# felipeagc/sycl-ray-tracer

Hardware: AMD Instinct MI355X
Metric: Mrays/s (higher is better)
Workload: dtype f32

## Files before the change

sycl-ray-tracer_amd/csrc/rt_bounce.h:

```cpp
#pragma once
#include "rt_device.h"

namespace rt {

RT_DEV f3 ray_dir(const RayState& r) { return mk3(h2f(r.dir[0]), h2f(r.dir[1]), h2f(r.dir[2])); }

template <bool FROM_TRAV = false, class Sink = NoSink>
RT_DEV bool shade_bounce(const SceneDev& S, uint32_t& rng, RayState& r, const Hit& h, f3& result, const Trav* T = nullptr, const ShadeTables* tab = nullptr,
                         long long* ck = nullptr, const Sink& sink = Sink{}) {
    f3 org = FROM_TRAV ? T->o : r.org;
    f3 dir = FROM_TRAV ? T->d : ray_dir(r);
    f3 att = mk3(h2f(r.att[0]), h2f(r.att[1]), h2f(r.att[2]));
    f3 rad = mk3(h2f(r.rad[0]), h2f(r.rad[1]), h2f(r.rad[2]));
    const bool done = FROM_TRAV ? shade_hit<true>(S, *tab, rng, h, org, dir, att, rad, result, ck, sink) : shade_hit<false>(S, ShadeTables{}, rng, h, org, dir, att, rad, result, nullptr, sink);
    r.org = org;
    r.dir[0] = f2h(dir.x), r.dir[1] = f2h(dir.y), r.dir[2] = f2h(dir.z);
    r.att[0] = f2h(att.x), r.att[1] = f2h(att.y), r.att[2] = f2h(att.z);
    r.rad[0] = f2h(rad.x), r.rad[1] = f2h(rad.y), r.rad[2] = f2h(rad.z);
    return done;
}

RT_DEV void origin_skip_none(const TravStack& stack) { *lds_at(skip_word_addr(stack)) = (int32_t)kSkipNone; }
RT_DEV SkipRec skip_entry(const SkipRec* at) {
    const u32x4* ep = reinterpret_cast<const u32x4*>(at);
    const u32x4 a = ep[0], b = ep[1];
    SkipRec e;
    e.ref = a.x, e.n[0] = __uint_as_float(a.y), e.n[1] = __uint_as_float(a.z), e.n[2] = __uint_as_float(a.w);
    e.p[0] = __uint_as_float(b.x), e.p[1] = __uint_as_float(b.y), e.p[2] = __uint_as_float(b.z), e.a = b.w;
    return e;
}
RT_DEV void origin_skip(const SceneDev& S, uint32_t tri, const Trav& T, const TravStack& stack) {
    const SkipRec e = skip_entry(S.skip + (tri == kNoTri ? 0u : tri));
    const float o[3] = {T.o.x, T.o.y, T.o.z}, d[3] = {T.d.x, T.d.y, T.d.z};
    const uint32_t w = origin_skip_word(e, o, d);
    *lds_at(skip_word_addr(stack)) = (int32_t)(tri == kNoTri ? kSkipNone : w);
}

RT_DEV bool roulette(uint32_t& rng, RayState& r) {
    const float qx = h2f(r.att[0]), qy = h2f(r.att[1]), qz = h2f(r.att[2]);
    const float p = __builtin_fminf(__builtin_fmaxf(__builtin_fmaxf(qx, __builtin_fmaxf(qy, qz)), 0.05f), 1.0f);
    const float u = rng_next(rng);
    if (!(u < p)) return false;
    r.att[0] = f2h(qx / p), r.att[1] = f2h(qy / p), r.att[2] = f2h(qz / p);
    return true;
}

}
```

sycl-ray-tracer_amd/csrc/rt_device.h:

```cpp
#pragma once
#include <hip/hip_runtime.h>

#include "../../include/rt_mi355x.h"
#include "rt_types.h"

namespace rt {

#define RT_DEV __device__ __forceinline__

struct f3 {
    float x, y, z;
};
RT_DEV f3 mk3(float x, float y, float z) { return f3{x, y, z}; }
RT_DEV f3 operator+(f3 a, f3 b) { return mk3(a.x + b.x, a.y + b.y, a.z + b.z); }
RT_DEV f3 operator-(f3 a, f3 b) { return mk3(a.x - b.x, a.y - b.y, a.z - b.z); }
RT_DEV f3 operator-(f3 a) { return mk3(-a.x, -a.y, -a.z); }
RT_DEV f3 operator*(f3 a, f3 b) { return mk3(a.x * b.x, a.y * b.y, a.z * b.z); }
RT_DEV f3 operator*(float s, f3 a) { return mk3(s * a.x, s * a.y, s * a.z); }
RT_DEV f3 operator*(f3 a, float s) { return mk3(a.x * s, a.y * s, a.z * s); }
RT_DEV float dot3(f3 a, f3 b) { return (a.x * b.x + a.y * b.y) + a.z * b.z; }
RT_DEV f3 cross3(f3 a, f3 b) {
    return mk3(a.y * b.z - a.z * b.y, a.z * b.x - a.x * b.z, a.x * b.y - a.y * b.x);
}
RT_DEV float rcp_rn(float x) {
    const uint32_t t = __float_as_uint(x) + __float_as_uint(x);
    const bool ok = t - 0x01000000u < 0xFC000000u;
    if (__builtin_expect(__builtin_amdgcn_ballot_w64(!ok) == 0ull, 1)) {
        const float y = __builtin_amdgcn_rcpf(x);
        return __builtin_fmaf(__builtin_fmaf(-x, y, 1.0f), y, y);
    }
    return 1.0f / x;
}
RT_DEV float inv_sqrt2(float x) {
    const bool ok = __float_as_uint(x) - 0x0C800000u < 0x73000000u;
    if (__builtin_expect(__builtin_amdgcn_ballot_w64(!ok) == 0ull, 1)) {
        const float r = __builtin_amdgcn_rsqf(x);
        float g = x * r, h = 0.5f * r;
        const float e = __builtin_fmaf(-h, g, 0.5f);
        g = __builtin_fmaf(g, e, g), h = __builtin_fmaf(h, e, h);
        const float s = __builtin_fmaf(__builtin_fmaf(-g, g, x), h, g);
        const float y = __builtin_amdgcn_rcpf(s);
        return __builtin_fmaf(__builtin_fmaf(-s, y, 1.0f), y, y);
    }
    return 1.0f / __builtin_sqrtf(x);
}
RT_DEV f3 normalize3(f3 a) {
    const float inv = inv_sqrt2(dot3(a, a));
    return mk3(a.x * inv, a.y * inv, a.z * inv);
}
RT_DEV float clamp01(float x) { return __builtin_fminf(__builtin_fmaxf(x, 0.0f), 1.0f); }

RT_DEV uint16_t f2h(float f) {
    asm("" : "+v"(f));
    _Float16 h = (_Float16)f;
    return __builtin_bit_cast(uint16_t, h);
}
RT_DEV float h2f(uint16_t b) { return (float)__builtin_bit_cast(_Float16, b); }

RT_DEV float rng_next(uint32_t& a) {
    uint32_t x = a;
    x ^= x << 13;
    x ^= x >> 17;
    x ^= x << 5;
    a = x;
    return (float)x * (1.0f / 4294967296.0f);
}
RT_DEV float rng_range(uint32_t& a, float mn, float mx) { return mn + (mx - mn) * rng_next(a); }
RT_DEV f3 rng_unit_vector(uint32_t& a) {
    float x = rng_range(a, -1.0f, 1.0f);
    float y = rng_range(a, -1.0f, 1.0f);
    float z = rng_range(a, -1.0f, 1.0f);
    return normalize3(mk3(x, y, z));
}

RT_DEV uint32_t pixel_seed(int x, int y, int w, int h, uint32_t seed_mode) {
    if (seed_mode == RT_SEED_MEGAKERNEL) {
        uint32_t h8 = (uint32_t)((h + 7) / 8) * 8u;
        return (uint32_t)x * h8 + (uint32_t)y;
    }
    return (uint32_t)x + (uint32_t)y * (uint32_t)w;
}

RT_DEV int tile_global_row(const TileDev& t, int local_row) {
    uint32_t strip = (uint32_t)local_row / t.strip_rows;
    uint32_t within = (uint32_t)local_row % t.strip_rows;
    return (int)((strip * t.world + t.rank) * t.strip_rows + within);
}

struct RayState {
    f3 org;
    uint16_t dir[3], att[3], rad[3];
};

RT_DEV RayState camera_ray(const CameraDev& c, int x, int y, uint32_t& rng) {
    f3 p00 = mk3(c.pixel00[0], c.pixel00[1], c.pixel00[2]);
    f3 du = mk3(c.du[0], c.du[1], c.du[2]);
    f3 dv = mk3(c.dv[0], c.dv[1], c.dv[2]);
    f3 center = mk3(c.center[0], c.center[1], c.center[2]);
    f3 pixel_center = (p00 + ((float)x * du)) + ((float)y * dv);
    float px = -0.5f + rng_next(rng);
    float py = -0.5f + rng_next(rng);
    f3 jitter = (px * du) + (py * dv);
    f3 pixel_sample = pixel_center + jitter;
    f3 d = pixel_sample - center;
    RayState r;
    r.org = center;
    r.dir[0] = f2h(d.x), r.dir[1] = f2h(d.y), r.dir[2] = f2h(d.z);
    r.att[0] = r.att[1] = r.att[2] = 0x3C00;
    r.rad[0] = r.rad[1] = r.rad[2] = 0;
    return r;
}

struct Hit {
    float t, u, v;
    uint32_t tri;
};

RT_DEV float dot3f(f3 a, f3 b) { return __builtin_fmaf(a.z, b.z, __builtin_fmaf(a.y, b.y, a.x * b.x)); }
RT_DEV f3 cross3f(f3 a, f3 b) {
    return mk3(__builtin_fmaf(a.y, b.z, -(a.z * b.y)), __builtin_fmaf(a.z, b.x, -(a.x * b.z)), __builtin_fmaf(a.x, b.y, -(a.y * b.x)));
}
RT_DEV void tri_test_regs(float4 a, float4 b, float2 c, f3 o, f3 d, Hit& best) {
    const f3 v0 = mk3(a.x, a.y, a.z), e1 = mk3(a.w, b.x, b.y), e2 = mk3(b.z, b.w, c.x);
    const uint32_t gidx = __float_as_uint(c.y);
    const f3 p = cross3f(d, e2);
    const float det = dot3f(e1, p);
    if (!(det != 0.0f)) return;
    const f3 tv = o - v0;
    const f3 q = cross3f(tv, e1);
    const float sgn = det < 0.0f ? -1.0f : 1.0f;
    const float un0 = dot3f(tv, p), vn0 = dot3f(d, q);
    const float un = un0 * sgn, vn = vn0 * sgn;
    if (!(un >= 0.0f && vn >= 0.0f && un + vn <= __builtin_fabsf(det))) return;
    const float inv = rcp_rn(det);
    const float t = dot3f(e2, q) * inv;
    if (!(t > kTNear)) return;
    if (t < best.t || (t == best.t && gidx < best.tri)) {
        best.t = t;
        best.u = un0 * inv;
        best.v = vn0 * inv;
        best.tri = gidx;
    }
}
typedef float f4a8 __attribute__((ext_vector_type(4), aligned(8)));
typedef float f2a8 __attribute__((ext_vector_type(2), aligned(8)));
RT_DEV float4 tri_ld4(const uint8_t* p) {
    const f4a8 v = *reinterpret_cast<const f4a8*>(p);
    return make_float4(v.x, v.y, v.z, v.w);
}
RT_DEV float2 tri_ld2(const uint8_t* p) {
    const f2a8 v = *reinterpret_cast<const f2a8*>(p);
    return make_float2(v.x, v.y);
}
RT_DEV void tri_test(const uint8_t* __restrict__ tr, f3 o, f3 d, Hit& best) {
    tri_test_regs(tri_ld4(tr), tri_ld4(tr + 16), tri_ld2(tr + 32), o, d, best);
}

constexpr int32_t kTravDone = (int32_t)0x80000000;
#if defined(RT_DEVELOPER_KNOBS) && defined(RT_VOTE_INNER) && defined(RT_VOTE_LEAF)
constexpr uint32_t kVoteInner = RT_VOTE_INNER, kVoteLeaf = RT_VOTE_LEAF;
#else
constexpr uint32_t kVoteInner = 3u, kVoteLeaf = 4u;
#endif
struct Trav {
    f3 o, d;
    float ix, iy, iz;
    float ox, oy, oz;
    Hit best;
    int32_t cur;
    uint32_t sp;
};

struct TravStack;
RT_DEV uint32_t stack_base(const TravStack& st);
RT_DEV void trav_begin(Trav& T, f3 o, f3 d, const TravStack& st) {
    T.o = o, T.d = d;
    T.best.t = __builtin_huge_valf();
    T.best.u = T.best.v = 0.0f;
    T.best.tri = kNoTri;
    const float kTiny = 1e-30f;
    const float dx = __builtin_fabsf(d.x) < kTiny ? __builtin_copysignf(kTiny, d.x) : d.x;
    const float dy = __builtin_fabsf(d.y) < kTiny ? __builtin_copysignf(kTiny, d.y) : d.y;
    const float dz = __builtin_fabsf(d.z) < kTiny ? __builtin_copysignf(kTiny, d.z) : d.z;
    T.ix = __builtin_amdgcn_rcpf(dx), T.iy = __builtin_amdgcn_rcpf(dy), T.iz = __builtin_amdgcn_rcpf(dz);
    T.ox = -o.x * T.ix, T.oy = -o.y * T.iy, T.oz = -o.z * T.iz;
    T.cur = 0;
    T.sp = stack_base(st);
}

constexpr int kLdsStack = 12;
typedef __attribute__((address_space(3))) int32_t lds_i32;
struct TravStack {
    uint32_t base;
    int32_t* spill;
    uint32_t pitch;
};
RT_DEV uint32_t stack_base(const TravStack& st) { return st.base + st.pitch; }
RT_DEV lds_i32* lds_at(uint32_t addr) { return (lds_i32*)(size_t)addr; }
RT_DEV uint32_t skip_word_addr(const TravStack& st) { return st.base + (uint32_t)kLdsStack * st.pitch; }
RT_DEV bool stack_shallow(const TravStack& st, const Trav& T, uint32_t pushes) { return T.sp <= st.base + ((uint32_t)kLdsStack - pushes) * st.pitch; }
RT_DEV void trav_pop_lds(Trav& T, const TravStack& st) {
    T.sp -= st.pitch;
    T.cur = *lds_at(T.sp);
}
RT_DEV void stk_push(const TravStack& st, Trav& T, int32_t v) {
    const uint32_t e = (T.sp - st.base) / st.pitch;
    if (e < (uint32_t)kLdsStack) *lds_at(T.sp) = v;
    else st.spill[e - (uint32_t)kLdsStack] = v;
    T.sp += st.pitch;
}
RT_DEV void trav_pop(Trav& T, const TravStack& st) {
    T.sp -= st.pitch;
    const uint32_t e = (T.sp - st.base) / st.pitch;
    T.cur = e < (uint32_t)kLdsStack ? *lds_at(T.sp) : st.spill[e - (uint32_t)kLdsStack];
}

typedef uint32_t u32x4 __attribute__((ext_vector_type(4)));
typedef uint32_t u32x2 __attribute__((ext_vector_type(2)));
typedef __attribute__((address_space(3))) u32x4 lds_u32x4;
struct TopTree {
    lds_u32x4* w0;
    lds_u32x4* w1;
    lds_u32x4* w2;
    lds_u32x4* ch;
    int32_t count;
};
RT_DEV void top_tree_fill(const SceneDev& S, u32x4* w0, u32x4* w1, u32x4* w2, u32x4* ch, int32_t count) {
    for (int32_t i = (int32_t)threadIdx.x; i < count; i += (int32_t)blockDim.x) {
        const u32x4* np = reinterpret_cast<const u32x4*>(S.nodes + i);
        w0[i] = np[0];
        w1[i] = np[1];
        w2[i] = np[2];
        ch[i] = np[3];
    }
}

typedef unsigned long long lmask;
RT_DEV lmask lanes(bool c) { return __builtin_amdgcn_ballot_w64(c); }
RT_DEV uint32_t lane_rank(lmask m) { return __builtin_amdgcn_mbcnt_hi((uint32_t)(m >> 32), __builtin_amdgcn_mbcnt_lo((uint32_t)m, 0u)); }
RT_DEV float sel(lmask m, float a, float b) {
    float d;
    asm("v_cndmask_b32_e64 %0, %1, %2, %3" : "=v"(d) : "v"(a), "v"(b), "s"(m));
    return d;
}
RT_DEV uint32_t sel(lmask m, uint32_t a, uint32_t b) {
    uint32_t d;
    asm("v_cndmask_b32_e64 %0, %1, %2, %3" : "=v"(d) : "v"(a), "v"(b), "s"(m));
    return d;
}
RT_DEV int32_t sel(lmask m, int32_t a, int32_t b) { return (int32_t)sel(m, (uint32_t)a, (uint32_t)b); }
RT_DEV bool in_mask(lmask m) { return __builtin_amdgcn_inverse_ballot_w64(m); }
RT_DEV uint32_t count(lmask m) { return (uint32_t)__builtin_popcountll(m); }

struct TravSigns {
    lmask nx, ny, nz;
};

RT_DEV float ub0(uint32_t w) { return (float)(w & 0xffu); }
RT_DEV float ub1(uint32_t w) { return (float)((w >> 8) & 0xffu); }
RT_DEV float ub2(uint32_t w) { return (float)((w >> 16) & 0xffu); }
RT_DEV float ub3(uint32_t w) { return (float)(w >> 24); }

struct WaveStats {
    uint32_t inner_steps = 0, inner_lanes = 0, leaf_steps = 0, leaf_lanes = 0;
    uint32_t shade_rounds = 0, shade_lanes = 0, live_lane_steps = 0, top_lanes = 0;
};
RT_DEV TravSigns trav_signs(const Trav& T) { return TravSigns{lanes(T.ix < 0.0f), lanes(T.iy < 0.0f), lanes(T.iz < 0.0f)}; }
template <bool SKIP = false, bool MISS_KEYS = false>
RT_DEV void trav_inner(const SceneDev& S, Trav& T, const TravStack& stack, const TopTree& top, const TravSigns& sg) {
    const float inf = __builtin_huge_valf();
    uint32_t skip = kSkipNone;
    if (SKIP) skip = (uint32_t)*lds_at(skip_word_addr(stack));
    float k0, k1, k2, k3;
    u32x4 w0, w1, w2, chw;
    if (T.cur < top.count * 64) {
        const uint32_t o = (uint32_t)T.cur >> 2;
        w0 = *(lds_u32x4*)(size_t)((uint32_t)(size_t)top.w0 + o), w1 = *(lds_u32x4*)(size_t)((uint32_t)(size_t)top.w1 + o);
        w2 = *(lds_u32x4*)(size_t)((uint32_t)(size_t)top.w2 + o), chw = *(lds_u32x4*)(size_t)((uint32_t)(size_t)top.ch + o);
    } else {
        asm volatile("global_load_dwordx4 %0, %4, %5\n\t"
                     "global_load_dwordx4 %1, %4, %5 offset:16\n\t"
                     "global_load_dwordx4 %2, %4, %5 offset:32\n\t"
                     "global_load_dwordx4 %3, %4, %5 offset:48"
                     : "=&v"(w0), "=&v"(w1), "=&v"(w2), "=&v"(chw)
                     : "v"((uint32_t)T.cur), "s"(S.nodes)
                     : "memory");
    }
    asm volatile("s_waitcnt vmcnt(1)" : "+v"(w0), "+v"(w1), "+v"(w2));
    const float ax = __uint_as_float(w0.w) * T.ix;
    const float ay = __uint_as_float(w2.z) * T.iy;
    const float az = __uint_as_float(w2.w) * T.iz;
    const float bx = __builtin_fmaf(__uint_as_float(w0.x), T.ix, T.ox);
    const float by = __builtin_fmaf(__uint_as_float(w0.y), T.iy, T.oy);
    const float bz = __builtin_fmaf(__uint_as_float(w0.z), T.iz, T.oz);
    const lmask nx = sg.nx, ny = sg.ny, nz = sg.nz;
    const uint32_t qnx = sel(nx, w1.x, w1.y), qfx = sel(nx, w1.y, w1.x);
    const uint32_t qny = sel(ny, w1.z, w1.w), qfy = sel(ny, w1.w, w1.z);
    const uint32_t qnz = sel(nz, w2.x, w2.y), qfz = sel(nz, w2.y, w2.x);
    lmask h0 = 0ull, h1 = 0ull, h2 = 0ull, h3 = 0ull;
#define RT_CHILD(K, H, CVT, CW)                                                                           \
    {                                                                                                    \
        const float tn = __builtin_fmaxf(__builtin_fmaxf(__builtin_fmaf(CVT(qnx), ax, bx), __builtin_fmaf(CVT(qny), ay, by)), \
                                         __builtin_fmaxf(__builtin_fmaf(CVT(qnz), az, bz), 0.0f));       \
         \
         \
         \
        const float fx = __builtin_fmaf(CVT(qfx), ax, bx), fy = __builtin_fmaf(CVT(qfy), ay, by), fz = __builtin_fmaf(CVT(qfz), az, bz); \
        const float tf = SKIP ? __builtin_fminf(__builtin_fminf(__builtin_fminf(fx, fy), fz), T.best.t)  \
                              : __builtin_fminf(__builtin_fminf(fx, fy), __builtin_fminf(fz, T.best.t)); \
        if (SKIP) H = lanes(tn <= tf) & lanes(CW != skip), K = MISS_KEYS ? sel(H, inf, tn) : tn;         \
        else K = sel(lanes(tn <= tf), inf, tn);                                                          \
    }
    if (SKIP) asm volatile("s_waitcnt vmcnt(0)" : "+v"(chw));
    RT_CHILD(k0, h0, ub0, chw.x)
    RT_CHILD(k1, h1, ub1, chw.y)
    RT_CHILD(k2, h2, ub2, chw.z)
    RT_CHILD(k3, h3, ub3, chw.w)
#undef RT_CHILD
#define RT_CE(KA, CA, KB, CB)                                                        \
    {                                                                               \
        const lmask sw = lanes(KB < KA);                                            \
        const float ka = sel(sw, KA, KB), kb = sel(sw, KB, KA);                     \
        const int32_t ca = sel(sw, CA, CB), cb = sel(sw, CB, CA);                   \
        KA = ka, KB = kb, CA = ca, CB = cb;                                         \
    }
    if (!SKIP) asm volatile("s_waitcnt vmcnt(0)" : "+v"(chw));
    int32_t c0 = (int32_t)chw.x, c1 = (int32_t)chw.y, c2 = (int32_t)chw.z, c3 = (int32_t)chw.w;
    if (SKIP) {
#define RT_CE_M(KA, HA, CA, KB, HB, CB)                                              \
    {                                                                               \
        const lmask sw = MISS_KEYS ? lanes(KB < KA) : HB & (~HA | lanes(KB < KA));  \
        KA = sel(sw, KA, KB);                                                       \
        const int32_t ca = sel(sw, CA, CB), cb = sel(sw, CB, CA);                   \
        CA = ca, CB = cb;                                                           \
        const lmask lo = HA | HB, hi = HA & HB;                                     \
        HA = lo, HB = hi;                                                           \
    }
        RT_CE_M(k0, h0, c0, k1, h1, c1)
        RT_CE_M(k2, h2, c2, k3, h3, c3)
        RT_CE_M(k0, h0, c0, k2, h2, c2)
#undef RT_CE_M
        if (lanes(!stack_shallow(stack, T, 3u)) == 0ull) {
            *lds_at(T.sp) = c3;
            T.sp = sel(h3, T.sp, T.sp + stack.pitch);
            *lds_at(T.sp) = c2;
            T.sp = sel(h2, T.sp, T.sp + stack.pitch);
            *lds_at(T.sp) = c1;
            T.sp = sel(h1, T.sp, T.sp + stack.pitch);
            if (in_mask(h0)) T.cur = c0;
            else trav_pop_lds(T, stack);
        } else {
            if (in_mask(h3)) stk_push(stack, T, c3);
            if (in_mask(h2)) stk_push(stack, T, c2);
            if (in_mask(h1)) stk_push(stack, T, c1);
            if (in_mask(h0)) T.cur = c0;
            else trav_pop(T, stack);
        }
        return;
    }
    RT_CE(k0, c0, k1, c1)
    RT_CE(k2, c2, k3, c3)
    RT_CE(k0, c0, k2, c2)
#undef RT_CE
    const bool descend = k0 < inf;
    if (lanes(!stack_shallow(stack, T, 3u)) == 0ull) {
        *lds_at(T.sp) = c3;
        T.sp = sel(lanes(k3 < inf), T.sp, T.sp + stack.pitch);
        *lds_at(T.sp) = c2;
        T.sp = sel(lanes(k2 < inf), T.sp, T.sp + stack.pitch);
        *lds_at(T.sp) = c1;
        T.sp = sel(lanes(k1 < inf), T.sp, T.sp + stack.pitch);
        if (descend) T.cur = c0;
        else trav_pop_lds(T, stack);
    } else {
        if (k3 < inf) stk_push(stack, T, c3);
        if (k2 < inf) stk_push(stack, T, c2);
        if (k1 < inf) stk_push(stack, T, c1);
        if (descend) T.cur = c0;
        else trav_pop(T, stack);
    }
}

template <bool BATCH>
RT_DEV void trav_leaf(const SceneDev& S, Trav& T, const TravStack& stack) {
    const uint32_t code = (uint32_t)~T.cur;
    const uint32_t first = code >> 2, rem = code & 3u;
    if (BATCH) {
        static_assert(kMaxLeafTris == 2 && kTriBytes == 40, "the whole-leaf step reads a leaf as 80 contiguous bytes");
        const uint8_t* p4 = S.tris + (size_t)first * kTriBytes;
        const float4 l0 = tri_ld4(p4), l1 = tri_ld4(p4 + 16), l2 = tri_ld4(p4 + 32), l3 = tri_ld4(p4 + 48), l4 = tri_ld4(p4 + 64);
        const bool two = rem != 0u;
        tri_test_regs(l0, l1, make_float2(l2.x, l2.y), T.o, T.d, T.best);
        if (__ballot(two) != 0ull) {
            if (two) tri_test_regs(make_float4(l2.z, l2.w, l3.x, l3.y), make_float4(l3.z, l3.w, l4.x, l4.y), make_float2(l4.z, l4.w), T.o, T.d, T.best);
        }
        if (lanes(!stack_shallow(stack, T, 0u)) == 0ull) trav_pop_lds(T, stack);
        else trav_pop(T, stack);
    } else {
        tri_test(S.tris + (size_t)first * kTriBytes, T.o, T.d, T.best);
        if (rem) T.cur = ~(int32_t)(((first + 1u) << 2) | (rem - 1u));
        else trav_pop(T, stack);
    }
}

struct TravClasses {
    lmask inner, leaf;
};
RT_DEV lmask trav_done(const Trav& T) { return lanes(T.cur == kTravDone); }
RT_DEV TravClasses trav_classes(const Trav& T) { return TravClasses{lanes(T.cur >= 0), lanes((uint32_t)T.cur > (uint32_t)kTravDone)}; }
RT_DEV TravClasses trav_classes(const Trav& T, lmask done) {
    const lmask inner = lanes(T.cur >= 0);
    return TravClasses{inner, lanes(true) & ~(inner | done)};
}
template <bool STATS = false, bool LEAF_BATCH = false, bool SKIP = false, bool MISS_KEYS = false>
RT_DEV uint32_t trav_step_wave(const SceneDev& S, Trav& T, const TravStack& stack, const TopTree& top, const TravSigns& sg, const TravClasses& c, WaveStats* ws = nullptr) {
    const uint32_t ni = count(c.inner), nl = count(c.leaf);
    if (ni * kVoteInner >= nl * kVoteLeaf && !(LEAF_BATCH && nl >= 64u)) {
        if (STATS && ni) ws->inner_steps++, ws->inner_lanes += ni, ws->top_lanes += count(c.inner & lanes(T.cur < (SKIP ? top.count : kTopNodes) * 64));
        if (in_mask(c.inner)) trav_inner<SKIP, MISS_KEYS>(S, T, stack, top, sg);
    } else {
        if (STATS) ws->leaf_steps++, ws->leaf_lanes += nl;
        if (in_mask(c.leaf)) trav_leaf<LEAF_BATCH>(S, T, stack);
    }
    return ni + nl;
}
template <bool STATS = false, bool LEAF_BATCH = false, bool SKIP = false, bool MISS_KEYS = false>
RT_DEV uint32_t trav_step_wave(const SceneDev& S, Trav& T, const TravStack& stack, const TopTree& top, const TravSigns& sg, WaveStats* ws = nullptr) {
    return trav_step_wave<STATS, LEAF_BATCH, SKIP, MISS_KEYS>(S, T, stack, top, sg, trav_classes(T), ws);
}

RT_DEV Hit intersect(const SceneDev& S, f3 o, f3 d, const TravStack& stack, const TopTree& top) {
    Trav T;
    trav_begin(T, o, d, stack);
    const TravSigns sg = trav_signs(T);
    while (trav_step_wave(S, T, stack, top, sg)) {}
    return T.best;
}

RT_DEV bool near_zero3(f3 e) {
    const float s = 1e-8f;
    return (__builtin_fabsf(e.x) < s) && (__builtin_fabsf(e.y) < s) && (__builtin_fabsf(e.z) < s);
}
RT_DEV float length_squared3(f3 v) {
    float l = __builtin_sqrtf(dot3(v, v));
    return l * l;
}
RT_DEV f3 reflect3(f3 v, f3 n) { return v - (2.0f * dot3(v, n)) * n; }
RT_DEV f3 refract3(f3 uv, f3 n, float etai_over_etat) {
    float cos_theta = __builtin_fminf(dot3(-uv, n), 1.0f);
    f3 r_out_perp = etai_over_etat * (uv + cos_theta * n);
    f3 r_out_parallel = (-__builtin_sqrtf(__builtin_fabsf(1.0f - length_squared3(r_out_perp)))) * n;
    return r_out_perp + r_out_parallel;
}
RT_DEV float schlick(float cosine, float ref_idx) {
    float r0 = (1.0f - ref_idx) / (1.0f + ref_idx);
    r0 = r0 * r0;
    float x = 1.0f - cosine;
    float x2 = x * x;
    float x5 = (x2 * x2) * x;
    return r0 + (1.0f - r0) * x5;
}
RT_DEV float unorm8_to_float(uint32_t b) {
    const float x = (float)b, r = 1.0f / 255.0f;
    const float q = x * r;
    return __builtin_fmaf(__builtin_fmaf(-q, 255.0f, x), r, q);
}

RT_DEV bool albedo_is_texture(const MatRec& m) { return (m.type == RT_MAT_DIFFUSE || m.type == RT_MAT_METALLIC) && m.tex_kind != RT_TEX_COLOR; }
RT_DEV uint32_t albedo_fetch(const SceneDev& S, const MatRec& m, float u, float v) {
    float fu = u - __builtin_floorf(u);
    float fv = v - __builtin_floorf(v);
    int iu = (int)__builtin_floorf(fu * 512.0f);
    int iv = (int)__builtin_floorf(fv * 512.0f);
    iu = iu < 0 ? 0 : (iu > 511 ? 511 : iu);
    iv = iv < 0 ? 0 : (iv > 511 ? 511 : iv);
    return *reinterpret_cast<const uint32_t*>(S.tex + (((size_t)m.tex_layer * 512u + (size_t)iv) * 512u + (size_t)iu) * 4u);
}
RT_DEV f3 albedo_decode(uint32_t texel) {
    return mk3(unorm8_to_float(texel & 0xffu), unorm8_to_float((texel >> 8) & 0xffu), unorm8_to_float((texel >> 16) & 0xffu));
}
RT_DEV f3 albedo(const SceneDev& S, const MatRec& m, float u, float v) {
    if (m.tex_kind == RT_TEX_COLOR) return mk3(m.color[0], m.color[1], m.color[2]);
    float fu = u - __builtin_floorf(u);
    float fv = v - __builtin_floorf(v);
    int iu = (int)__builtin_floorf(fu * 512.0f);
    int iv = (int)__builtin_floorf(fv * 512.0f);
    iu = iu < 0 ? 0 : (iu > 511 ? 511 : iu);
    iv = iv < 0 ? 0 : (iv > 511 ? 511 : iv);
    const uint32_t texel = *reinterpret_cast<const uint32_t*>(
        S.tex + (((size_t)m.tex_layer * 512u + (size_t)iv) * 512u + (size_t)iu) * 4u);
    return mk3(unorm8_to_float(texel & 0xffu), unorm8_to_float((texel >> 8) & 0xffu), unorm8_to_float((texel >> 16) & 0xffu));
}

template <bool PRE = false>
RT_DEV bool scatter(const SceneDev& S, const MatRec& m, uint32_t& rng, f3 dir, f3 normal, float u, float v,
                    f3& out_dir, f3& out_att, uint32_t texel = 0) {
    if (m.type == RT_MAT_DIFFUSE || m.type == RT_MAT_METALLIC) {
        const bool diffuse = m.type == RT_MAT_DIFFUSE;
        const f3 unit = rng_unit_vector(rng);
        const f3 reflected = reflect3(dir, normal);
        const f3 base = diffuse ? normal : reflected;
        const f3 offs = diffuse ? unit : m.roughness * unit;
        out_dir = base + offs;
        if (diffuse && near_zero3(dir)) out_dir = normal;
        if (PRE) out_att = m.tex_kind == RT_TEX_COLOR ? mk3(m.color[0], m.color[1], m.color[2]) : albedo_decode(texel);
        else out_att = albedo(S, m, u, v);
        return diffuse ? true : dot3(out_dir, normal) > 0.0f;
    }
    if (m.type == RT_MAT_DIELECTRIC) {
        out_att = mk3(1.0f, 1.0f, 1.0f);
        bool front_face = dot3(dir, normal) < 0.0f;
        f3 n = front_face ? normal : -normal;
        float ratio = front_face ? (1.0f / m.ior) : m.ior;
        f3 unit_direction = normalize3(dir);
        float cos_theta = __builtin_fminf(dot3(-unit_direction, n), 1.0f);
        float sin_theta = __builtin_sqrtf(1.0f - cos_theta * cos_theta);
        bool reflect_it = ratio * sin_theta > 1.0f;
        if (!reflect_it) reflect_it = schlick(cos_theta, ratio) > rng_range(rng, 0.0f, 1.0f);
        out_dir = reflect_it ? reflect3(unit_direction, n) : refract3(unit_direction, n, ratio);
        return true;
    }
    out_dir = mk3(0.0f, 0.0f, 0.0f);
    out_att = mk3(0.0f, 0.0f, 0.0f);
    return false;
}

struct ShadeTables {
    lds_u32x4* nm;
    lds_u32x4* mat;
    uint32_t n_nm, n_mat;
};
RT_DEV void shade_tables_fill(const SceneDev& S, u32x4* nm, u32x4* mat) {
    const u32x4* in = reinterpret_cast<const u32x4*>(S.inst);
    for (uint32_t i = threadIdx.x; i < S.lds_nm * 3u; i += blockDim.x) nm[i] = in[i];
    for (uint32_t i = threadIdx.x; i < S.lds_mats; i += blockDim.x) {
        const u32x4* mp = reinterpret_cast<const u32x4*>(S.mats + i);
        const u32x4 m0 = mp[0], m1 = mp[1], m2 = mp[2];
        u32x4 a, b;
        a.x = m0.x | (m0.y << 8) | (m1.y << 16), a.y = m0.z, a.z = m0.w, a.w = m1.x;
        b.x = m1.z, b.y = m1.w, b.z = m2.x, b.w = m0.x == RT_MAT_DIELECTRIC ? m2.z : m2.y;
        mat[2u * i] = a, mat[2u * i + 1u] = b;
    }
}

#ifdef RT_ROUND_STAMPS
#define RT_STAMP_AFTER(ck, i, VAL)                                                     \
    do {                                                                              \
        if (ck) {                                                                     \
            asm volatile("" ::"v"(VAL));                                              \
            const long long n_ = (long long)__builtin_readcyclecounter();             \
            (ck)[i] += n_ - (ck)[7];                                                  \
            (ck)[7] = n_;                                                             \
        }                                                                             \
    } while (0)
#else
#define RT_STAMP_AFTER(ck, i, VAL) do { } while (0)
#endif
struct NoSink {};
template <class Sink> struct is_no_sink { static constexpr bool value = false; };
template <> struct is_no_sink<NoSink> { static constexpr bool value = true; };
template <bool USE_TAB = false, class Sink = NoSink>
RT_DEV bool shade_hit(const SceneDev& S, const ShadeTables& tab, uint32_t& rng, const Hit& h, f3& org, f3& dir, f3& att, f3& rad, f3& result,
                      long long* ck = nullptr, const Sink& sink = Sink{}) {
    if (h.tri == kNoTri) {
        if constexpr (is_no_sink<Sink>::value) result = att * (mk3(S.sky[0], S.sky[1], S.sky[2]) + rad);
        else sink(att * (mk3(S.sky[0], S.sky[1], S.sky[2]) + rad));
        return true;
    }
    const float4* sp = reinterpret_cast<const float4*>(S.shade + h.tri);
    const float4 s0 = sp[0], s1 = sp[1], s2 = sp[2], s3 = sp[3];
    const f3 d = normalize3(dir);
    const f3 n0 = mk3(s0.x, s0.y, s0.z), n1 = mk3(s0.w, s1.x, s1.y), n2 = mk3(s1.z, s1.w, s2.x);
    const float uv0x = s2.y, uv0y = s2.z, uv1x = s2.w, uv1y = s3.x, uv2x = s3.y, uv2y = s3.z;
    const uint32_t iw = __float_as_uint(s3.w);
    RT_STAMP_AFTER(ck, 1, iw);
    bool lds = false;
    if (USE_TAB) lds = __builtin_amdgcn_ballot_w64(!((iw & kPackedInstMask) < tab.n_nm && (iw >> kPackedInstBits) < tab.n_mat)) == 0ull;
    MatRec mat;
    if (USE_TAB && __builtin_expect(lds, 1)) {
        const uint32_t at = (iw >> kPackedInstBits) * 2u;
        const u32x4 a = tab.mat[at], b = tab.mat[at + 1u];
        mat.type = a.x & 0xffu, mat.tex_kind = (a.x >> 8) & 0xffu, mat.tex_layer = a.x >> 16;
        mat.color[0] = __uint_as_float(a.y), mat.color[1] = __uint_as_float(a.z), mat.color[2] = __uint_as_float(a.w);
        mat.emissive[0] = __uint_as_float(b.x), mat.emissive[1] = __uint_as_float(b.y), mat.emissive[2] = __uint_as_float(b.z);
        mat.roughness = mat.ior = __uint_as_float(b.w);
    } else {
        const InstRec* inst = S.inst + (S.packed_mat ? (iw & kPackedInstMask) : iw);
        const u32x4* mp = reinterpret_cast<const u32x4*>(S.mats + (S.packed_mat ? (iw >> kPackedInstBits) : inst->material));
        const u32x4 m0 = mp[0], m1 = mp[1], m2 = mp[2];
        mat.type = m0.x, mat.tex_kind = m0.y, mat.color[0] = __uint_as_float(m0.z), mat.color[1] = __uint_as_float(m0.w);
        mat.color[2] = __uint_as_float(m1.x), mat.tex_layer = m1.y, mat.emissive[0] = __uint_as_float(m1.z), mat.emissive[1] = __uint_as_float(m1.w);
        mat.emissive[2] = __uint_as_float(m2.x), mat.roughness = __uint_as_float(m2.y), mat.ior = __uint_as_float(m2.z);
    }
    const float bx = h.u, by = h.v;
    const float w = (1.0f - bx) - by;
    const float tu = (w * uv0x + bx * uv1x) + by * uv2x;
    const float tv = (w * uv0y + bx * uv1y) + by * uv2y;
    uint32_t texel;
    {
        float fu = tu - __builtin_floorf(tu);
        float fv = tv - __builtin_floorf(tv);
        int iu = (int)__builtin_floorf(fu * 512.0f);
        int iv = (int)__builtin_floorf(fv * 512.0f);
        iu = iu < 0 ? 0 : (iu > 511 ? 511 : iu);
        iv = iv < 0 ? 0 : (iv > 511 ? 511 : iv);
        const uint8_t* ta = S.tex + (((size_t)mat.tex_layer * 512u + (size_t)iv) * 512u + (size_t)iu) * 4u;
        if (!albedo_is_texture(mat)) ta = reinterpret_cast<const uint8_t*>(sp);
        texel = *reinterpret_cast<const uint32_t*>(ta);
        RT_STAMP_AFTER(ck, 2, ta);
    }
    const bool emits = mat.type == RT_MAT_DIFFUSE || mat.type == RT_MAT_METALLIC;
    rad = rad + (emits ? mk3(mat.emissive[0], mat.emissive[1], mat.emissive[2]) : mk3(0.0f, 0.0f, 0.0f));
    const f3 vn = normalize3((w * n0 + bx * n1) + by * n2);
    float nm[9];
    if (USE_TAB && __builtin_expect(lds, 1)) {
        const uint32_t at = (iw & kPackedInstMask) * 3u;
        const u32x4 a = tab.nm[at], b = tab.nm[at + 1u];
        const uint32_t c = *reinterpret_cast<__attribute__((address_space(3))) const uint32_t*>(tab.nm + at + 2u);
        nm[0] = __uint_as_float(a.x), nm[1] = __uint_as_float(a.y), nm[2] = __uint_as_float(a.z), nm[3] = __uint_as_float(a.w);
        nm[4] = __uint_as_float(b.x), nm[5] = __uint_as_float(b.y), nm[6] = __uint_as_float(b.z), nm[7] = __uint_as_float(b.w);
        nm[8] = __uint_as_float(c);
    } else {
        const InstRec* inst = S.inst + (S.packed_mat ? (iw & kPackedInstMask) : iw);
        u32x4 a, b;
        uint32_t c;
        asm volatile("global_load_dwordx4 %0, %3, off\n\t"
                     "global_load_dwordx4 %1, %3, off offset:16\n\t"
                     "global_load_dword %2, %3, off offset:32\n\t"
                     "s_waitcnt vmcnt(0)"
                     : "=&v"(a), "=&v"(b), "=&v"(c)
                     : "v"(inst)
                     : "memory");
        nm[0] = __uint_as_float(a.x), nm[1] = __uint_as_float(a.y), nm[2] = __uint_as_float(a.z), nm[3] = __uint_as_float(a.w);
        nm[4] = __uint_as_float(b.x), nm[5] = __uint_as_float(b.y), nm[6] = __uint_as_float(b.z), nm[7] = __uint_as_float(b.w);
        nm[8] = __uint_as_float(c);
    }
    const f3 g = mk3((nm[0] * vn.x + nm[3] * vn.y) + nm[6] * vn.z, (nm[1] * vn.x + nm[4] * vn.y) + nm[7] * vn.z,
                     (nm[2] * vn.x + nm[5] * vn.y) + nm[8] * vn.z);
    const f3 normal = normalize3(g);
    RT_STAMP_AFTER(ck, 3, normal.x);
    f3 sdir, satt;
#ifdef RT_SCATTER_PRIO
    __builtin_amdgcn_s_setprio(RT_SCATTER_PRIO);
#endif
    const bool scattered = scatter<true>(S, mat, rng, d, normal, tu, tv, sdir, satt, texel);
    RT_STAMP_AFTER(ck, 4, satt.x);
    if (scattered) {
        org = mk3(org.x + dir.x * h.t, org.y + dir.y * h.t, org.z + dir.z * h.t);
        dir = sdir;
        att = att * satt;
        return false;
    }
    if constexpr (is_no_sink<Sink>::value) result = att * rad;
    else sink(att * rad);
    return true;
}

RT_DEV uint8_t to_unorm8(float c) { return (uint8_t)__builtin_rintf(clamp01(c) * 255.0f); }

#define RT_TRAVERSAL_LDS(BLOCK) RT_TRAVERSAL_LDS_(BLOCK, kTopNodes, 0)
#define RT_TRAVERSAL_LDS_SKIP(BLOCK, ON)                                                               \
    RT_TRAVERSAL_LDS_(BLOCK, (ON) ? kTopNodes - (int)(BLOCK) / 16 : kTopNodes, (ON) ? 1 : 0)           \
    if (ON) lds_stack[kLdsStack * (BLOCK) + threadIdx.x] = (int32_t)kSkipNone;
#define RT_TRAVERSAL_LDS_(BLOCK, NTOP, EXTRA)                                                          \
    __shared__ u32x4 top_all[4 * (NTOP)];  \
    u32x4 *const top_w0 = top_all, *const top_w1 = top_all + (NTOP), *const top_w2 = top_all + 2 * (NTOP), *const top_ch = top_all + 3 * (NTOP); \
    __shared__ int32_t lds_stack[(kLdsStack + (EXTRA)) * (BLOCK)];                                     \
    int32_t spill[kStackSize - kLdsStack];                                                             \
    const int32_t top_count = (int32_t)S.n_nodes < (NTOP) ? (int32_t)S.n_nodes : (NTOP);               \
    top_tree_fill(S, top_w0, top_w1, top_w2, top_ch, top_count);                                       \
    __syncthreads();                                                                                   \
    const TopTree top{(lds_u32x4*)top_w0, (lds_u32x4*)top_w1, (lds_u32x4*)top_w2, (lds_u32x4*)top_ch, top_count}; \
    const TravStack stack{(uint32_t)(size_t)(lds_i32*)(lds_stack + threadIdx.x), spill, 4u * (BLOCK)}; \
    lds_stack[threadIdx.x] = kTravDone;

#define RT_SHADE_LDS                                                                                   \
    __shared__ u32x4 shade_nm[3 * kLdsNm], shade_mat[2 * kLdsMats];                                    \
    shade_tables_fill(S, shade_nm, shade_mat);                                                         \
    const ShadeTables tab{(lds_u32x4*)shade_nm, (lds_u32x4*)shade_mat, S.lds_nm, S.lds_mats};


}
```

sycl-ray-tracer_amd/csrc/rt_kernels.h:

```cpp
#pragma once
#include <cstddef>

#include "rt_bounce.h"
#include "rt_device.h"
#include "rt_launch.h"

namespace rt {

RT_DEV void queue_store(const QueueDev& q, uint32_t slot, uint32_t id, const RayState& r) {
    q.org_id[slot] = make_float4(r.org.x, r.org.y, r.org.z, __uint_as_float(id));
    q.a[slot] = make_uint2((uint32_t)r.dir[0] | ((uint32_t)r.dir[1] << 16), (uint32_t)r.dir[2] | ((uint32_t)r.att[0] << 16));
    q.b[slot] = make_uint2((uint32_t)r.att[1] | ((uint32_t)r.att[2] << 16), (uint32_t)r.rad[0] | ((uint32_t)r.rad[1] << 16));
    q.c[slot] = r.rad[2];
}
RT_DEV uint32_t queue_load(const QueueDev& q, uint32_t slot, RayState& r) {
    const float4 o = q.org_id[slot];
    const uint2 a = q.a[slot], b = q.b[slot];
    const uint16_t c = q.c[slot];
    r.org = mk3(o.x, o.y, o.z);
    r.dir[0] = (uint16_t)a.x, r.dir[1] = (uint16_t)(a.x >> 16), r.dir[2] = (uint16_t)a.y;
    r.att[0] = (uint16_t)(a.y >> 16), r.att[1] = (uint16_t)b.x, r.att[2] = (uint16_t)(b.x >> 16);
    r.rad[0] = (uint16_t)b.y, r.rad[1] = (uint16_t)(b.y >> 16), r.rad[2] = c;
    return __float_as_uint(o.w);
}

RT_DEV uint32_t wave_sum_u32(uint32_t v) {
#pragma unroll
    for (int off = 32; off > 0; off >>= 1) v += __shfl_down(v, off, 64);
    return v;
}
RT_DEV unsigned long long wave_sum_u64(uint32_t v) {
    return (unsigned long long)wave_sum_u32(v & 0xFFFFu) + ((unsigned long long)wave_sum_u32(v >> 16) << 16);
}

RT_DEV void wave_stats_flush(const WaveStats& ws, unsigned long long* stats_out) {
    atomicAdd(stats_out + 0, (unsigned long long)ws.inner_steps), atomicAdd(stats_out + 1, (unsigned long long)ws.inner_lanes);
    atomicAdd(stats_out + 2, (unsigned long long)ws.leaf_steps), atomicAdd(stats_out + 3, (unsigned long long)ws.leaf_lanes);
    atomicAdd(stats_out + 4, (unsigned long long)ws.shade_rounds), atomicAdd(stats_out + 5, (unsigned long long)ws.shade_lanes);
    atomicAdd(stats_out + 6, (unsigned long long)ws.live_lane_steps), atomicAdd(stats_out + 7, (unsigned long long)ws.top_lanes);
}

template <class F, class I> RT_DEV void pixel_end(const F* sum_r, const F* sum_g, const F* sum_b, float n, I o, float* __restrict__ out_f32, uint8_t* __restrict__ out_u8) {
    const f3 c = mk3(__builtin_sqrtf(*sum_r / n), __builtin_sqrtf(*sum_g / n), __builtin_sqrtf(*sum_b / n));
    if (out_f32) reinterpret_cast<float4*>(out_f32)[o] = make_float4(c.x, c.y, c.z, 1.0f);
    if (out_u8)
        reinterpret_cast<uint32_t*>(out_u8)[o] = (uint32_t)to_unorm8(c.x) | ((uint32_t)to_unorm8(c.y) << 8) | ((uint32_t)to_unorm8(c.z) << 16) | 0xff000000u;
}
RT_DEV uint32_t stream_lane_row(uint32_t r, uint32_t strip_rows, uint32_t n_lanes, uint32_t lane_index) {
    return ((r / strip_rows) * n_lanes + lane_index) * strip_rows + r % strip_rows;
}

#ifndef RT_ROUND_PRIO
#define RT_ROUND_PRIO 0
#endif
#if defined(RT_DEVELOPER_KNOBS) && defined(RT_MEGA_UNROLL)
constexpr int kMegaUnroll = RT_MEGA_UNROLL;
#else
constexpr int kMegaUnroll = 4;
#endif
#if defined(RT_DEVELOPER_KNOBS) && defined(RT_FINISH_UNROLL)
constexpr int kFinishUnroll = RT_FINISH_UNROLL;
#else
constexpr int kFinishUnroll = 3;
#endif
#ifndef RT_MEGA_SHADE_PCT
#define RT_MEGA_SHADE_PCT 75
#endif
constexpr uint32_t kMegaShadePct = RT_MEGA_SHADE_PCT;
constexpr uint32_t kMegaRefill = 1;
template <int UNROLL>
struct RefillPolicy {
    uint32_t w = (kMegaRefill - 1u) << 28;
    RT_DEV uint32_t threshold() const { return (w >> 28) + 1u; }
    RT_DEV void stepped() {
        if (((w >> 17) & 0x7FFu) != 0x7FFu) w += 1u << 17;
    }
    RT_DEV void round(bool finished) {
        w += ((uint32_t)__popcll(__ballot(finished)) << 5) + 1u;
        if ((w & 31u) == 0u) {
            const uint32_t ended = ((w >> 5) & 0xFFFu) - 1u, steps = ((w >> 17) & 0x7FFu) * (uint32_t)UNROLL;
            const uint32_t num = 320u * ended, den = 160u + steps;
            const uint32_t t = num < 4u * den ? 1u : num < 9u * den ? 2u : num < 16u * den ? 3u : num < 25u * den ? 4u : num < 36u * den ? 5u
                               : num < 64u * den ? 6u : num < 100u * den ? 8u : num < 144u * den ? 10u : num < 256u * den ? 12u : 16u;
            w = (t - 1u) << 28;
        }
    }
};
template <uint32_t OFF> RT_DEV uint32_t frame_u32(const MegaFrame* f) {
    uint32_t v;
    asm volatile("s_load_dword %0, %1, %2\n\t"
                 "s_waitcnt lgkmcnt(0)"
                 : "=&s"(v)
                 : "s"(f), "i"(OFF));
    return v;
}
template <uint32_t OFF> RT_DEV unsigned long long frame_u64(const MegaFrame* f) {
    unsigned long long v;
    asm volatile("s_load_dwordx2 %0, %1, %2\n\t"
                 "s_waitcnt lgkmcnt(0)"
                 : "=&s"(v)
                 : "s"(f), "i"(OFF));
    return v;
}
RT_DEV CameraDev frame_camera(const MegaFrame* f, int32_t width, int32_t height) {
    static_assert(offsetof(MegaFrame, cam) == 0 && offsetof(CameraDev, dv) + sizeof(CameraDev::dv) == 48, "the camera's twelve floats lead MegaFrame");
    u32x4 a, b, c;
    asm volatile("s_load_dwordx4 %0, %3, 0x0\n\t"
                 "s_load_dwordx4 %1, %3, 0x10\n\t"
                 "s_load_dwordx4 %2, %3, 0x20\n\t"
                 "s_waitcnt lgkmcnt(0)"
                 : "=&s"(a), "=&s"(b), "=&s"(c)
                 : "s"(f));
    CameraDev cam;
    cam.center[0] = __uint_as_float(a.x), cam.center[1] = __uint_as_float(a.y), cam.center[2] = __uint_as_float(a.z);
    cam.pixel00[0] = __uint_as_float(a.w), cam.pixel00[1] = __uint_as_float(b.x), cam.pixel00[2] = __uint_as_float(b.y);
    cam.du[0] = __uint_as_float(b.z), cam.du[1] = __uint_as_float(b.w), cam.du[2] = __uint_as_float(c.x);
    cam.dv[0] = __uint_as_float(c.y), cam.dv[1] = __uint_as_float(c.z), cam.dv[2] = __uint_as_float(c.w);
    cam.width = width, cam.height = height;
    return cam;
}
RT_DEV CameraDev frame_camera_and_seed(const MegaFrame* f, int32_t width, int32_t height, uint32_t& seed_add) {
    u32x4 a, b, c;
    uint32_t s;
    asm volatile("s_load_dwordx4 %0, %4, 0x0\n\t"
                 "s_load_dwordx4 %1, %4, 0x10\n\t"
                 "s_load_dwordx4 %2, %4, 0x20\n\t"
                 "s_load_dword %3, %4, %5\n\t"
                 "s_waitcnt lgkmcnt(0)"
                 : "=&s"(a), "=&s"(b), "=&s"(c), "=&s"(s)
                 : "s"(f), "i"((uint32_t)offsetof(MegaFrame, seed_add)));
    CameraDev cam;
    cam.center[0] = __uint_as_float(a.x), cam.center[1] = __uint_as_float(a.y), cam.center[2] = __uint_as_float(a.z);
    cam.pixel00[0] = __uint_as_float(a.w), cam.pixel00[1] = __uint_as_float(b.x), cam.pixel00[2] = __uint_as_float(b.y);
    cam.du[0] = __uint_as_float(b.z), cam.du[1] = __uint_as_float(b.w), cam.du[2] = __uint_as_float(c.x);
    cam.dv[0] = __uint_as_float(c.y), cam.dv[1] = __uint_as_float(c.z), cam.dv[2] = __uint_as_float(c.w);
    cam.width = width, cam.height = height;
    seed_add = s;
    return cam;
}
struct SliceNow {
    u32x4 head;
    u32x2 cuts;
};
RT_DEV SliceNow frame_slices(const MegaFrame* f) {
    static_assert(offsetof(SliceDev, tag0) == offsetof(SliceDev, state) + 8 && offsetof(SliceDev, shift) == offsetof(SliceDev, state) + 12, "SliceNow::head");
    SliceNow n;
    asm volatile("s_load_dwordx4 %0, %2, %3\n\t"
                 "s_load_dwordx2 %1, %2, %4\n\t"
                 "s_waitcnt lgkmcnt(0)"
                 : "=&s"(n.head), "=&s"(n.cuts)
                 : "s"(f), "i"((uint32_t)offsetof(MegaFrame, sl.state)), "i"((uint32_t)offsetof(MegaFrame, sl.cuts)));
    return n;
}
RT_DEV uint32_t frame_slice_bound(const MegaFrame* f, uint32_t j) {
    uint32_t v;
    const uint32_t at = (uint32_t)__builtin_amdgcn_readfirstlane((int)((uint32_t)offsetof(MegaFrame, sl.bound) + 4u * j));
    asm volatile("s_load_dword %0, %1, %2\n\t"
                 "s_waitcnt lgkmcnt(0)"
                 : "=&s"(v)
                 : "s"(f), "s"(at));
    return v;
}
RT_DEV u32x4* frame_carry(const MegaFrame* f) { return (u32x4*)frame_u64<offsetof(MegaFrame, carry)>(f); }
RT_DEV uint32_t frame_carry_total(const MegaFrame* f) { return frame_u32<offsetof(MegaFrame, carry_total)>(f); }
RT_DEV uint32_t frame_n_blocks(const MegaFrame* f) { return frame_u32<offsetof(MegaFrame, n_blocks)>(f); }
RT_DEV const uint32_t* frame_blocks(const MegaFrame* f) { return (const uint32_t*)frame_u64<offsetof(MegaFrame, blocks)>(f); }
RT_DEV const uint32_t* frame_block_count(const MegaFrame* f) { return (const uint32_t*)frame_u64<offsetof(MegaFrame, block_count)>(f); }
RT_DEV uint32_t frame_slice_wait_cap(const MegaFrame* f) { return frame_u32<offsetof(MegaFrame, sl.wait_cap)>(f); }
RT_DEV u32x4 carry_word(float r, float g, float b, uint32_t rng) {
    u32x4 w;
    w.x = __float_as_uint(r), w.y = __float_as_uint(g), w.z = __float_as_uint(b), w.w = rng;
    return w;
}
typedef __attribute__((address_space(3))) uint32_t lds_u32_word;
RT_DEV bool slice_wait_count(lds_u32_word* looks, const MegaFrame* f) {
    __builtin_amdgcn_s_sleep(127);
    const uint32_t n = *looks + 1u;
    *looks = n;
    return n == frame_slice_wait_cap(f) + 1u;
}
RT_DEV bool slice_wait_over(const lds_u32_word* looks, const MegaFrame* f) { return *looks > frame_slice_wait_cap(f); }
RT_DEV lds_u32_word* slice_looks_word(const void __attribute__((address_space(3))) * lane_slot, const void __attribute__((address_space(3))) * planes) {
    uint32_t a = (uint32_t)(size_t)lane_slot;
    asm volatile("" : "+v"(a));
    const uint32_t base = (uint32_t)(size_t)planes;
    return (lds_u32_word*)(size_t)(base + 3u * kMegaBlock * 4u + (((a - base) >> 6) & ~3u));
}
template <int STATS, bool SLICED, int CARRY = 0>
__global__ void __launch_bounds__(kMegaBlock, kMegaWaves) k_megakernel(SceneDev S, const MegaFrame* frame, int32_t width, int32_t height, TileDev tile,
                                                    uint32_t max_depth, uint32_t spp, uint32_t seed_mode, uint32_t rr_start, float* __restrict__ out_f32,
                                                    uint8_t* __restrict__ out_u8,
                                                    unsigned long long* __restrict__ ray_counter,
                                                    unsigned long long* __restrict__ stats_out, uint32_t n_slices) {
    WaveStats ws;
    long long t_begin = 0, t_mark = 0, t_trav = 0, t_shade = 0;
    long long ck[8] = {0, 0, 0, 0, 0, 0, 0, 0};
    if (STATS) t_begin = t_mark = (long long)__builtin_readcyclecounter();
    unsigned long long wall_begin = 0, wall_exhausted = 0;
    if (STATS >= 2) wall_begin = wall_clock64();
    const uint32_t tiles_x = (uint32_t)(width + 7) >> 3, tiles_y = (uint32_t)(tile.local_rows + 7) >> 3;
    const uint32_t n_slots = (CARRY == 3 ? frame_n_blocks(frame) : tiles_x * tiles_y) * 64u;
    const int lane = (int)(threadIdx.x & 63u);
    uint32_t* pixel_cursor = reinterpret_cast<uint32_t*>(ray_counter + 1);
    int x = 0, gy = 0;
    uint32_t pix = 0;
    uint32_t rng = 0, s = 0, depth = 0;
    unsigned long long wave_rays = 0;
    __shared__ float color_lds[3 * kMegaBlock + (SLICED ? kMegaBlock / 64 : 0)];
    typedef __attribute__((address_space(3))) float lds_f32;
    lds_f32* const color_r = (lds_f32*)color_lds + threadIdx.x;
    lds_f32* const color_g = color_r + kMegaBlock;
    lds_f32* const color_b = color_g + kMegaBlock;
    RayState r{};
    Trav T;
    if (SLICED) *slice_looks_word(color_r, (lds_f32*)color_lds) = 0u;
    RT_SHADE_LDS
    RT_TRAVERSAL_LDS_SKIP(kMegaBlock, true)
    T.cur = kTravDone;
    constexpr uint32_t kPend = 0x40000000u;
    bool live = false;
    RefillPolicy<kMegaUnroll> refill;
    bool exhausted = false;
    uint32_t slice_j = 0;
    auto state_rsrc = [&](const SliceNow& n) {
        return __builtin_amdgcn_make_buffer_rsrc((void*)(((unsigned long long)n.head.y << 32) | n.head.x), 0, (int)((uint32_t)tile.local_rows * (uint32_t)width * 32u), 0x00020000);
    };
    auto take_slot = [&](uint32_t p, uint32_t first) {
        uint32_t t = p >> 6;
        if constexpr (CARRY == 3) t = frame_blocks(frame)[t];
        x = (int)((t % tiles_x) * 8u + (p & 7u));
        const int ly = (int)((t / tiles_x) * 8u + ((p >> 3) & 7u));
        gy = tile_global_row(tile, ly);
        pix = (uint32_t)ly * (uint32_t)width + (uint32_t)x;
        if (x < width && ly < tile.local_rows && gy < height) {
            s = first;
            if (!SLICED || first == 0) {
                depth = 0;
                if constexpr (CARRY >= 2) {
                    const u32x4 c = frame_carry(frame)[pix];
                    rng = c.w;
                    *color_r = __uint_as_float(c.x), *color_g = __uint_as_float(c.y), *color_b = __uint_as_float(c.z);
                    r = camera_ray(frame_camera(frame, width, height), x, gy, rng);
                } else {
                    uint32_t seed_add;
                    const CameraDev cam = frame_camera_and_seed(frame, width, height, seed_add);
                    rng = pixel_seed(x, gy, width, height, seed_mode) + seed_add;
                    *color_r = 0.0f, *color_g = 0.0f, *color_b = 0.0f;
                    r = camera_ray(cam, x, gy, rng);
                }
                trav_begin(T, r.org, ray_dir(r), stack);
                origin_skip_none(stack);
            } else {
                depth = kPend;
            }
            live = true;
        }
    };
    {
        const uint32_t n_waves = gridDim.x * (kMegaBlock / 64u);
        if (n_slots <= n_waves * 64u && n_slices == 1u) {
            const uint32_t p = (uint32_t)lane * n_waves + blockIdx.x * (kMegaBlock / 64u) + (threadIdx.x >> 6);
            if (p < n_slots) take_slot(p, 0u);
            exhausted = true;
            if (STATS >= 2) wall_exhausted = wall_clock64();
        }
    }
    for (;;) {
        if (!exhausted) {
            const unsigned long long idle_m = __ballot(!live);
            const uint32_t cnt = (uint32_t)__popcll(idle_m);
            if (cnt >= refill.threshold()) {
                const uint32_t w = SLICED ? SliceCursor::claim_width(cnt, n_slots) : cnt;
                uint32_t base = 0;
                if (lane == 0) base = atomicAdd(pixel_cursor, w);
                base = (uint32_t)__builtin_amdgcn_readfirstlane((int)base);
                uint32_t first_here = 0, first_next = 0;
                if (SLICED) {
                    slice_j = SliceCursor::advance(slice_j, n_slices, base, n_slots);
                    if (slice_j) first_here = frame_slice_bound(frame, slice_j - 1u);
                    first_next = frame_slice_bound(frame, slice_j);
                }
                const uint32_t total_slots = SLICED ? n_slots * n_slices : n_slots;
                const uint32_t rank = __builtin_amdgcn_mbcnt_hi((uint32_t)(idle_m >> 32), __builtin_amdgcn_mbcnt_lo((uint32_t)idle_m, 0u));
                const uint32_t q = base + rank;
                if (!live && q < total_slots && rank < w) {
                    const SliceSlot m = SLICED ? SliceCursor::map(q, slice_j, n_slots, first_here, first_next) : SliceSlot{q, 0u};
                    take_slot(m.slot, m.first);
                }
                if (base + w >= total_slots) {
                    exhausted = true;
                    if (STATS >= 2) wall_exhausted = wall_clock64();
                }
            }
        }
        const uint32_t n_live = (uint32_t)__popcll(__ballot(live));
        if (n_live == 0) {
            if (exhausted) break;
            continue;
        }
        if (STATS) t_mark = (long long)__builtin_readcyclecounter();
        const TravSigns sg = trav_signs(T);
        const uint32_t n_rays = SLICED ? (uint32_t)__popcll(__ballot(live && depth < kPend)) : n_live;
        const lmask live_m = lanes(live);
        const uint32_t shade_at = n_rays * kMegaShadePct + (n_live - n_rays) * 100u;
        for (;;) {
            const lmask done = trav_done(T);
            if (count(done & live_m) * 100u >= shade_at) break;
            if (STATS >= 2) ws.live_lane_steps += n_live * (uint32_t)kMegaUnroll;
            if (STATS == 1) ws.inner_steps += (uint32_t)kMegaUnroll;
            refill.stepped();
            (void)trav_step_wave<(STATS >= 2), true, true, true>(S, T, stack, top, sg, trav_classes(T, done), &ws);
#pragma unroll
            for (int k = 1; k < kMegaUnroll; ++k) (void)trav_step_wave<(STATS >= 2), true, true, true>(S, T, stack, top, sg, &ws);
        }
        if (STATS) {
            ws.shade_rounds++;
            if (STATS >= 2) ws.shade_lanes += (uint32_t)__popcll(__ballot(live && T.cur == kTravDone));
            const long long now = (long long)__builtin_readcyclecounter();
            t_trav += now - t_mark, t_mark = now;
        }
        __builtin_amdgcn_s_setprio(RT_ROUND_PRIO);
#ifdef RT_ROUND_STAMPS
        if (STATS >= 2) ck[7] = (long long)__builtin_readcyclecounter();
#endif
        bool pixel_finished = false;
        bool bounced = false;
        {
            const unsigned long long traced = __ballot(live && T.cur == kTravDone && depth < kPend);
            wave_rays += (unsigned long long)__popcll(traced);
            if (SLICED && traced == 0ull && __ballot(live && depth < kPend) == 0ull && slice_wait_count(slice_looks_word(color_r, (lds_f32*)color_lds), frame) && lane == 0) atomicMax(ray_counter + 2, 1ull);
        }
        if (live && T.cur == kTravDone) {
            bool start = false;
            if (SLICED && depth >= kPend) {
                const SliceNow sn = frame_slices(frame);
                const auto rsrc = state_rsrc(sn);
                const uint32_t at = pix * 32u, tag = sn.head.z + s;
                const u32x4 w0 = __builtin_amdgcn_raw_buffer_load_b128(rsrc, (int)at, 0, 16 );
                const u32x4 w1 = __builtin_amdgcn_raw_buffer_load_b128(rsrc, (int)(at + 16u), 0, 16 );
                if ((w0.y == tag && w0.w == tag && w1.y == tag && w1.w == tag) || slice_wait_over(slice_looks_word(color_r, (lds_f32*)color_lds), frame)) {
                    *color_r = __uint_as_float(w0.x), *color_g = __uint_as_float(w0.z), *color_b = __uint_as_float(w1.x);
                    rng = w1.z;
                    start = true;
                }
            } else {
                f3 res;
                const auto add = [color_r, color_g, color_b](const f3& c) { *color_r = *color_r + c.x, *color_g = *color_g + c.y, *color_b = *color_b + c.z; };
                bool done;
                if (SLICED) {
                    done = shade_bounce<true>(S, rng, r, T.best, res, &T, &tab, STATS >= 2 ? ck : nullptr, add);
                } else {
                    done = shade_bounce<true>(S, rng, r, T.best, res, &T, &tab, STATS >= 2 ? ck : nullptr);
                    if (done) add(res);
                }
#ifdef RT_TAIL_PRIO
                __builtin_amdgcn_s_setprio(RT_TAIL_PRIO);
#endif
                depth++;
                bool killed = false;
                if (rr_start && !done && depth >= rr_start && depth < max_depth) killed = !roulette(rng, r);
                if (done || killed || depth == max_depth) {
                    s++;
                    bool handed = false;
                    SliceNow sn{};
                    if (SLICED) {
                        sn = frame_slices(frame);
                        const unsigned long long cuts = ((unsigned long long)sn.cuts.y << 32) | sn.cuts.x;
                        const uint32_t sh = sn.head.w;
                        handed = s < spp && (s & ((1u << sh) - 1u)) == 0u && ((cuts >> (s >> sh)) & 1ull) != 0ull;
                    }
                    if (SLICED && handed) {
                        live = false, pixel_finished = true;
                        const auto rsrc = state_rsrc(sn);
                        const uint32_t at = pix * 32u, tag = sn.head.z + s;
                        u32x4 w0, w1;
                        w0.x = __float_as_uint(*color_r), w0.y = tag, w0.z = __float_as_uint(*color_g), w0.w = tag;
                        w1.x = __float_as_uint(*color_b), w1.y = tag, w1.z = rng, w1.w = tag;
                        __builtin_amdgcn_raw_buffer_store_b128(w0, rsrc, (int)at, 0, 16 );
                        __builtin_amdgcn_raw_buffer_store_b128(w1, rsrc, (int)(at + 16u), 0, 16 );
                    } else if (s < spp) {
                        start = true;
                    } else {
                        live = false, pixel_finished = true;
                        float n;
                        if constexpr (CARRY == 3)
                            n = (float)frame_block_count(frame)[(pix / (uint32_t)width >> 3) * tiles_x + ((uint32_t)x >> 3)];
                        else
                            n = (float)(CARRY == 2 ? frame_carry_total(frame) : spp);
                        pixel_end(color_r, color_g, color_b, n, pix, out_f32, out_u8);
                        if constexpr (CARRY != 0) frame_carry(frame)[pix] = carry_word(*color_r, *color_g, *color_b, rng);
                    }
                } else {
                    bounced = true;
                }
            }
            if (start) {
                depth = 0;
                int cx = x, cy = gy;
                asm volatile("" : "+v"(cx), "+v"(cy));
                r = camera_ray(frame_camera(frame, width, height), cx, cy, rng);
            }
            if (live && depth < kPend) {
                const uint32_t from = bounced ? T.best.tri : kNoTri;
                trav_begin(T, r.org, ray_dir(r), stack);
                origin_skip(S, from, T, stack);
            }
            RT_STAMP_AFTER((STATS >= 2 ? ck : nullptr), 5, T.ox);
        }
        refill.round(pixel_finished);
        if (STATS) t_shade += (long long)__builtin_readcyclecounter() - t_mark;
        __builtin_amdgcn_s_setprio(2);
    }
    if (lane == 0 && wave_rays) atomicAdd(ray_counter, wave_rays);
    if (STATS && lane == 0) {
        wave_stats_flush(ws, stats_out);
        const unsigned long long dur = (unsigned long long)((long long)__builtin_readcyclecounter() - t_begin);
        atomicAdd(stats_out + 8, dur), atomicMax(stats_out + 9, dur), atomicAdd(stats_out + 10, 1ull);
        atomicAdd(stats_out + 11, (unsigned long long)t_trav), atomicAdd(stats_out + 12, (unsigned long long)t_shade);
        if (STATS >= 2) {
            atomicMin(stats_out + 13, wall_begin);
            if (wall_exhausted) atomicMin(stats_out + 14, wall_exhausted);
            atomicMax(stats_out + 15, (unsigned long long)wall_clock64());
        }
#ifdef RT_ROUND_STAMPS
        for (int i = 1; i <= 5; ++i) atomicAdd(stats_out + 15 + i, (unsigned long long)ck[i]);
#endif
    }
}

__global__ void __launch_bounds__(256) k_fill_black(uint32_t n_local, float* __restrict__ out_f32, uint8_t* __restrict__ out_u8) {
    const uint32_t i = blockIdx.x * 256u + threadIdx.x;
    if (i >= n_local) return;
    if (out_f32) reinterpret_cast<float4*>(out_f32)[i] = make_float4(0.0f, 0.0f, 0.0f, 1.0f);
    if (out_u8) reinterpret_cast<uint32_t*>(out_u8)[i] = 0xff000000u;
}

__global__ void __launch_bounds__(256) k_wf_init(const CameraDev* __restrict__ camp, TileDev tile, uint32_t seed_mode, uint32_t seed_add, uint32_t n_local,
                                                  uint32_t* __restrict__ rng, float4* __restrict__ accum) {
    const uint32_t i = blockIdx.x * 256u + threadIdx.x;
    if (i >= n_local) return;
    const CameraDev cam = *camp;
    const int x = (int)(i % (uint32_t)cam.width), ly = (int)(i / (uint32_t)cam.width);
    const int gy = tile_global_row(tile, ly);
    rng[i] = pixel_seed(x, gy, cam.width, cam.height, seed_mode) + seed_add;
    accum[i] = make_float4(0.0f, 0.0f, 0.0f, 0.0f);
}
__global__ void __launch_bounds__(256) k_wf_init_carry(uint32_t n_local, uint32_t width, uint32_t strip_rows, uint32_t n_lanes, uint32_t lane_index,
                                                        const u32x4* __restrict__ carry, uint32_t* __restrict__ rng, float4* __restrict__ accum) {
    const uint32_t i = blockIdx.x * 256u + threadIdx.x;
    if (i >= n_local) return;
    const uint32_t x = i % width, row = stream_lane_row(i / width, strip_rows, n_lanes, lane_index);
    const u32x4 c = carry[(size_t)row * width + x];
    rng[i] = c.w;
    accum[i] = make_float4(__uint_as_float(c.x), __uint_as_float(c.y), __uint_as_float(c.z), 0.0f);
}

__global__ void __launch_bounds__(256) k_wf_generate(const CameraDev* __restrict__ camp, TileDev tile, uint32_t n_local,
                                                      uint32_t* __restrict__ rng, QueueDev q,
                                                      uint32_t* __restrict__ count_out, uint32_t spread, const uint32_t* __restrict__ tile_order) {
    const uint32_t i = blockIdx.x * 256u + threadIdx.x;
    if (i == 0) *count_out = n_local;
    if (i >= n_local) return;
    const CameraDev cam = *camp;
    const uint32_t nw = n_local >> 6;
    uint32_t id = spread && nw * 64u == n_local ? (i & 63u) * nw + (i >> 6) : i;
    if (tile_order) {
        const uint32_t t = tile_order[i >> 6], w = i & 63u, tiles_x = (uint32_t)cam.width >> 3;
        id = ((t / tiles_x) * 8u + (w >> 3)) * (uint32_t)cam.width + (t % tiles_x) * 8u + (w & 7u);
    }
    const int x = (int)(id % (uint32_t)cam.width), ly = (int)(id / (uint32_t)cam.width);
    const int gy = tile_global_row(tile, ly);
    uint32_t st = rng[id];
    const RayState r = gy < cam.height ? camera_ray(cam, x, gy, st) : RayState{};
    rng[id] = st;
    queue_store(q, i, id, r);
}

__global__ void __launch_bounds__(64) k_wf_tile_cost(const uint8_t* __restrict__ cost, uint32_t width, uint32_t n_tiles, uint32_t* __restrict__ key) {
    const uint32_t t = blockIdx.x, w = threadIdx.x, tiles_x = width >> 3;
    if (t >= n_tiles) return;
    uint32_t v = cost[((t / tiles_x) * 8u + (w >> 3)) * width + (t % tiles_x) * 8u + (w & 7u)];
#pragma unroll
    for (int off = 32; off > 0; off >>= 1) v += __shfl_down(v, off, 64);
    if (w == 0) key[t] = v >> 2;
}
constexpr uint32_t kOrderBins = 64u * 255u / 4u + 1u;
__global__ void __launch_bounds__(1024) k_wf_order_tiles(const uint32_t* __restrict__ key, uint32_t n_tiles, uint32_t* __restrict__ order) {
    __shared__ uint32_t bin[kOrderBins];
    for (uint32_t i = threadIdx.x; i < kOrderBins; i += 1024u) bin[i] = 0;
    __syncthreads();
    for (uint32_t t = threadIdx.x; t < n_tiles; t += 1024u) atomicAdd(&bin[key[t] < kOrderBins ? key[t] : kOrderBins - 1u], 1u);
    __syncthreads();
    if (threadIdx.x == 0) {
        uint32_t run = 0;
        for (uint32_t k = kOrderBins; k-- > 0;) {
            const uint32_t c = bin[k];
            bin[k] = run;
            run += c;
        }
    }
    __syncthreads();
    for (uint32_t t = threadIdx.x; t < n_tiles; t += 1024u) order[atomicAdd(&bin[key[t] < kOrderBins ? key[t] : kOrderBins - 1u], 1u)] = t;
}


constexpr uint32_t kExtendRefill = 16;
template <bool STATS>
__global__ void __launch_bounds__(kExtendBlock, kExtendWaves) k_wf_extend(SceneDev S, QueueDev qin, float4* __restrict__ hits,
                                                                    const uint32_t* __restrict__ count_in,
                                                                    uint32_t* __restrict__ cursor,
                                                                    unsigned long long* __restrict__ stats_out) {
    WaveStats ws;
    const uint32_t n = *count_in;
    const uint32_t lane = threadIdx.x & 63u;
    constexpr uint32_t kWavesPerBlock = kExtendBlock / 64;
    const uint32_t wave_id = blockIdx.x * kWavesPerBlock + (threadIdx.x >> 6);
    const uint32_t n_waves = gridDim.x * kWavesPerBlock;
    RT_TRAVERSAL_LDS(kExtendBlock)
    Trav T;
    T.cur = kTravDone;
    bool has = false;
    bool pending = false;
    float4 pend_o = make_float4(0.0f, 0.0f, 0.0f, 0.0f);
    uint2 pend_a = make_uint2(0u, 0u);
    uint32_t slot = 0;
    uint32_t chunk_pos = wave_id * kExtendChunk;
    uint32_t chunk_end = chunk_pos + kExtendChunk < n ? chunk_pos + kExtendChunk : n;
    bool exhausted = chunk_pos >= n;
    if (exhausted) return;
    TravSigns sg{0ull, 0ull, 0ull};
    for (;;) {
        const bool any_pending = __ballot(pending) != 0ull;
        if (pending) {
            const f3 d = mk3(h2f((uint16_t)pend_a.x), h2f((uint16_t)(pend_a.x >> 16)), h2f((uint16_t)pend_a.y));
            trav_begin(T, mk3(pend_o.x, pend_o.y, pend_o.z), d, stack);
            pending = false;
        }
        if (any_pending) sg = trav_signs(T);
        const bool need = T.cur == kTravDone;
        const unsigned long long need_m = __ballot(need);
        const uint32_t cnt = (uint32_t)__popcll(need_m);
        if (cnt >= kExtendRefill || cnt == 64u) {
            if (STATS) ws.shade_rounds++, ws.shade_lanes += cnt;
            if (need && has) {
                hits[slot] = make_float4(T.best.t, T.best.u, T.best.v, __uint_as_float(T.best.tri));
                has = false;
            }
            if (!exhausted) {
                if (chunk_pos == chunk_end) {
                    uint32_t base = 0;
                    if (lane == 0) base = atomicAdd(cursor, kExtendChunk);
                    base = (uint32_t)__builtin_amdgcn_readfirstlane((int)base) + n_waves * kExtendChunk;
                    if (base >= n) exhausted = true;
                    chunk_pos = base;
                    chunk_end = base + kExtendChunk < n ? base + kExtendChunk : n;
                }
                if (!exhausted) {
                    const uint32_t avail = chunk_end - chunk_pos;
                    const uint32_t take = cnt < avail ? cnt : avail;
                    const uint32_t rank = lane_rank(need_m);
                    if (need && rank < take) {
                        slot = chunk_pos + rank;
                        pend_o = qin.org_id[slot];
                        pend_a = qin.a[slot];
                        pending = true;
                        has = true;
                    }
                    chunk_pos += take;
                }
            }
        }
        if (__ballot(T.cur != kTravDone) == 0ull) {
            if (__ballot(pending) != 0ull) continue;
            if (exhausted) break;
            continue;
        }
        if (STATS) ws.live_lane_steps += (uint32_t)__popcll(__ballot(has));
        (void)trav_step_wave<STATS, true>(S, T, stack, top, sg, &ws);
    }
    if (STATS && lane == 0) wave_stats_flush(ws, stats_out);
}

RT_DEV uint32_t reorder_key(const SceneDev& S, const RayState& r) {
    auto cell = [&](float p, int a) {
        const int c = (int)((p - S.cell_lo[a]) * S.cell_scale[a]);
        return (uint32_t)(c < 0 ? 0 : (c > 3 ? 3 : c));
    };
    const uint32_t cx = cell(r.org.x, 0), cy = cell(r.org.y, 1), cz = cell(r.org.z, 2);
    const uint32_t morton = (cx & 1u) | ((cy & 1u) << 1) | ((cz & 1u) << 2) | ((cx >> 1) << 3) | ((cy >> 1) << 4) | ((cz >> 1) << 5);
    const uint32_t oct = ((uint32_t)(r.dir[0] >> 15) & 1u) | (((uint32_t)(r.dir[1] >> 15) & 1u) << 1) | (((uint32_t)(r.dir[2] >> 15) & 1u) << 2);
    return (oct << 6) | morton;
}

RT_DEV uint32_t block_scan_256(uint32_t v, uint32_t* wave_sums , uint32_t* total) {
    const uint32_t lane = threadIdx.x & 63u, wave = threadIdx.x >> 6;
    uint32_t incl = v;
#pragma unroll
    for (int off = 1; off < 64; off <<= 1) {
        const uint32_t o = __shfl_up(incl, off, 64);
        if ((int)lane >= off) incl += o;
    }
    if (lane == 63u) wave_sums[wave] = incl;
    __syncthreads();
    uint32_t base = 0;
    for (uint32_t w = 0; w < wave; ++w) base += wave_sums[w];
    *total = wave_sums[0] + wave_sums[1] + wave_sums[2] + wave_sums[3];
    return base + incl - v;
}

template <bool REORDER, bool MATSORT>
__global__ void __launch_bounds__(256) k_wf_shade(SceneDev S, QueueDev qin, QueueDev qout, const float4* __restrict__ hits,
                                                   uint32_t* __restrict__ rng, float4* __restrict__ accum,
                                                   const uint32_t* __restrict__ count_in,
                                                   uint32_t* __restrict__ count_out, int last_depth, int rr_active) {
    __shared__ uint32_t wave_total[4];
    __shared__ uint32_t block_base;
    __shared__ uint32_t bins[REORDER ? 512 : 1];
    __shared__ uint32_t perm[MATSORT ? 256 : 1];
    __shared__ uint32_t kind_count[MATSORT ? 8 : 1];
    const uint32_t n = *count_in;
    uint32_t i = blockIdx.x * 256u + threadIdx.x;
    if (blockIdx.x * 256u >= n) return;
    if (MATSORT) {
        uint32_t kind = 7u;
        if (i < n) {
            const uint32_t tri = __float_as_uint(hits[i].w);
            kind = 0u;
            if (tri != kNoTri) {
                const uint32_t iw = S.shade[tri].instance;
                kind = 1u + (S.mats[S.packed_mat ? (iw >> kPackedInstBits) : S.inst[iw].material].type & 3u);
            }
        }
        if (threadIdx.x < 8u) kind_count[threadIdx.x] = 0u;
        __syncthreads();
        const uint32_t rank_in_kind = atomicAdd(&kind_count[kind], 1u);
        __syncthreads();
        uint32_t before = 0;
        for (uint32_t k = 0; k < kind; ++k) before += kind_count[k];
        perm[before + rank_in_kind] = i;
        __syncthreads();
        i = perm[threadIdx.x];
    }
    bool survive = false;
    RayState r{};
    uint32_t id = 0;
    if (i < n) {
        id = queue_load(qin, i, r);
        const float4 hr = hits[i];
        Hit hit;
        hit.t = hr.x, hit.u = hr.y, hit.v = hr.z, hit.tri = __float_as_uint(hr.w);
        uint32_t st = rng[id];
        f3 res;
        const bool done = shade_bounce(S, st, r, hit, res);
        if (done) {
            float4 acc = accum[id];
            acc.x = acc.x + clamp01(res.x), acc.y = acc.y + clamp01(res.y), acc.z = acc.z + clamp01(res.z);
            accum[id] = acc;
        } else {
            survive = !last_depth;
            if (rr_active && survive) survive = roulette(st, r);
        }
        rng[id] = st;
    }
    if (REORDER) {
        bins[threadIdx.x] = 0u, bins[threadIdx.x + 256u] = 0u;
        __syncthreads();
        uint32_t key = 0, rank_in_bin = 0;
        if (survive) {
            key = reorder_key(S, r);
            rank_in_bin = atomicAdd(&bins[key], 1u);
        }
        __syncthreads();
        const uint32_t b0 = bins[2u * threadIdx.x], b1 = bins[2u * threadIdx.x + 1u];
        uint32_t total = 0;
        const uint32_t off = block_scan_256(b0 + b1, wave_total, &total);
        if (threadIdx.x == 0) block_base = total ? atomicAdd(count_out, total) : 0u;
        __syncthreads();
        bins[2u * threadIdx.x] = off, bins[2u * threadIdx.x + 1u] = off + b0;
        __syncthreads();
        if (survive) queue_store(qout, block_base + bins[key] + rank_in_bin, id, r);
        return;
    }
    const unsigned long long mask = __ballot(survive);
    const uint32_t lane = threadIdx.x & 63u, wave = threadIdx.x >> 6;
    const uint32_t prefix = lane_rank(mask);
    if (lane == 0) wave_total[wave] = (uint32_t)__popcll(mask);
    __syncthreads();
    if (threadIdx.x == 0) {
        const uint32_t total = wave_total[0] + wave_total[1] + wave_total[2] + wave_total[3];
        block_base = total ? atomicAdd(count_out, total) : 0u;
    }
    __syncthreads();
    if (survive) {
        uint32_t slot = block_base + prefix;
        for (uint32_t w = 0; w < wave; ++w) slot += wave_total[w];
        queue_store(qout, slot, id, r);
    }
}

constexpr uint32_t kRqIdleCap = 1u << 26;
constexpr uint32_t kNoRay = 0xFFFFFFFFu;
constexpr uint32_t kRqEmpty = 0xFFFFFFFFu, kRqStage = 96u, kRqFlush = 32u, kRqClaim = 16u;
static_assert(kRqFlush + 64u <= kRqStage, "a whole wave of new entries must fit behind an unflushed stage");
RT_DEV unsigned long long rq_load64(const unsigned long long* p) { return __hip_atomic_load(p, __ATOMIC_RELAXED, __HIP_MEMORY_SCOPE_AGENT); }
RT_DEV void rq_store64(unsigned long long* p, unsigned long long v) { __hip_atomic_store(p, v, __ATOMIC_RELAXED, __HIP_MEMORY_SCOPE_AGENT); }

template <bool STATS, bool REQ, bool LIMIT = false, bool SLICED = false, bool CARRY = false, bool BLOCKS = false>
__global__ void __launch_bounds__(kMegaBlock, kMegaWaves) k_wf_finish(SceneDev S, const CameraDev* __restrict__ camp, TileDev tile, QueueDev qin,
                                                                    const uint32_t* __restrict__ count_in, uint32_t* __restrict__ cursor,
                                                                    uint32_t* __restrict__ rng_buf, float4* __restrict__ accum,
                                                                    unsigned long long* __restrict__ extra_rays, uint32_t first_depth, uint32_t max_depth,
                                                                    uint32_t n_samples, uint32_t rr_start,
                                                                    unsigned long long* __restrict__ stats_out, FinishRequeue fq, uint32_t chunk_slots, uint8_t* __restrict__ cost_out,
                                                                    QueueDev qout = QueueDev{}, uint32_t* __restrict__ count_out = nullptr, uint32_t bounce_limit = 0,
                                                                    uint32_t qflags = 0, const MegaFrame* slices = nullptr, uint32_t n_slices = 1) {
    static_assert(!(REQ && LIMIT), "the dynamic queue and the per-bounce hand-over are different schedules");
    static_assert(!(SLICED && (REQ || LIMIT)), "pixel slices belong to the one-launch schedule");
    static_assert(!CARRY || SLICED, "only the sliced schedule keeps a pixel's sums outside the accumulator");
    static_assert(!BLOCKS || CARRY, "a block continuation is a continuation");
    constexpr uint32_t kPend = 0x40000000u;
    const bool holes = (qflags & 1u) != 0u;
    __shared__ unsigned long long out_word;
    __shared__ uint32_t out_exited;
    if (LIMIT && threadIdx.x == 0) out_word = (unsigned long long)kOutBlock, out_exited = 0u;
    __shared__ uint32_t slot_lost;
    if (SLICED && threadIdx.x == 0) slot_lost = 0u;
    WaveStats ws;
    const uint32_t n = *count_in;
    const uint32_t lane = threadIdx.x & 63u;
    constexpr uint32_t kWavesPerBlock = kMegaBlock / 64;
    const uint32_t wave_id = blockIdx.x * kWavesPerBlock + (threadIdx.x >> 6);
    const uint32_t n_waves = gridDim.x * kWavesPerBlock;
    RT_SHADE_LDS
    constexpr bool kSkip = !LIMIT;
    RT_TRAVERSAL_LDS_SKIP(kMegaBlock, kSkip)
    __shared__ unsigned long long rq_stage_mem[REQ ? kWavesPerBlock * kRqStage : 1u];
    typedef __attribute__((address_space(3))) unsigned long long lds_u64_t;
    lds_u64_t* stage = (lds_u64_t*)rq_stage_mem + (threadIdx.x >> 6) * kRqStage;
    uint32_t staged = 0, stale = 0;
    uint32_t idle_polls = 0;
    const uint32_t total_entries = REQ ? n * (n_samples - 1u) : 0u;
    const auto accum_rsrc = __builtin_amdgcn_make_buffer_rsrc((void*)accum, 0, (int)(n * 16u), 0x00020000);
    __shared__ uint32_t xg_lds[SLICED ? 1u : kMegaBlock];
    typedef __attribute__((address_space(3))) uint32_t lds_u32_t;
    auto xg_word = [&]() {
        uint32_t a = stack.base;
        asm volatile("" : "+v"(a));
        return (lds_u32_t*)(size_t)(a - (uint32_t)(size_t)(lds_i32*)lds_stack + (uint32_t)(size_t)(lds_u32_t*)xg_lds);
    };
    const bool xg_packed = !SLICED && camp->width < 65536 && camp->height < 65536;
    __shared__ float sum_lds[SLICED ? 3u * kMegaBlock + kMegaBlock / 64u : 1u];
    typedef __attribute__((address_space(3))) float lds_f32_t;
    lds_f32_t* const sum_r = (lds_f32_t*)sum_lds + (SLICED ? threadIdx.x : 0u);
    lds_f32_t* const sum_g = sum_r + (SLICED ? kMegaBlock : 0u);
    lds_f32_t* const sum_b = sum_g + (SLICED ? kMegaBlock : 0u);
    if (SLICED) *slice_looks_word(sum_r, (lds_f32_t*)sum_lds) = 0u;
    bool chunk_dq = false;
    bool drained = false;
    bool waiting = false;
    Trav T;
    T.cur = kTravDone;
    bool live = false;
    RefillPolicy<kFinishUnroll> refill;
    RayState r{};
    uint32_t id = 0, rng = 0, depth = 0;
    unsigned long long wave_rays = 0;
    uint32_t samples_left = 0;
    bool first_counted = false;
    const bool tail_guided = LIMIT && (chunk_slots >> 31) != 0u;
    const uint32_t static_pct = (chunk_slots >> 16) & 0x7Fu;
    chunk_slots &= 0xFFFFu;
    uint32_t first_slots = chunk_slots;
    if (SLICED) first_slots = 0;
    if (tail_guided) {
        const uint32_t per_wave = (uint32_t)(((unsigned long long)n * static_pct / 100u) / (n_waves ? n_waves : 1u));
        first_slots = per_wave < 64u ? 64u : (per_wave & ~63u);
    }
    uint32_t seen = n_waves * first_slots;
    const uint32_t inv_waves = tail_guided ? 0x10000u / (n_waves ? n_waves : 1u) + 1u : 0u;
    const uint32_t n_total = SLICED ? n * n_slices : n;
    uint32_t slice_j = 0;
    uint32_t chunk_pos = wave_id * first_slots;
    uint32_t chunk_end = chunk_pos + first_slots < n_total ? chunk_pos + first_slots : n_total;
    bool exhausted = chunk_pos >= n_total;
    auto state_rsrc = [&](const SliceNow& sn) {
        const uint32_t n_state = BLOCKS ? (uint32_t)tile.local_rows * (uint32_t)camp->width : n;
        return __builtin_amdgcn_make_buffer_rsrc((void*)(((unsigned long long)sn.head.y << 32) | sn.head.x), 0, (int)(n_state * 32u), 0x00020000);
    };
    auto leave = [&]() {
        if (!LIMIT) return;
        uint32_t order = 0;
        if (lane == 0) order = atomicAdd(&out_exited, 1u);
        order = (uint32_t)__builtin_amdgcn_readfirstlane((int)order);
        if (order + 1u != kWavesPerBlock) return;
        const unsigned long long w = out_word;
        const uint32_t used = (uint32_t)w, base = (uint32_t)(w >> 32);
        for (uint32_t i = used + lane; i < kOutBlock; i += 64u) qout.org_id[base + i] = make_float4(0.0f, 0.0f, 0.0f, __uint_as_float(kNoRay));
    };
    if (exhausted) {
        if (!REQ) {
            leave();
            return;
        }
        chunk_pos = chunk_end = 0;
    }
    auto flush = [&]() {
        uint32_t t = 0;
        if (lane == 0) t = atomicAdd(fq.ctl + 0, staged);
        t = (uint32_t)__builtin_amdgcn_readfirstlane((int)t);
        asm volatile("s_waitcnt vmcnt(0)" ::: "memory");
        for (uint32_t i = lane; i < staged; i += 64u)
            if (t + i < fq.capacity) rq_store64(fq.entries + t + i, stage[i]);
        if (lane == 0 && t + staged > fq.capacity) __hip_atomic_store(fq.error, 2u, __ATOMIC_RELAXED, __HIP_MEMORY_SCOPE_AGENT);
        staged = 0;
    };
    for (;;) {
        if (REQ && waiting && samples_left != kRqEmpty) {
            const uint32_t e = samples_left;
            id = e & 0xFFFFFFu, samples_left = (e >> 24) + 1u;
            const CameraDev cam = *camp;
            const int x = (int)(id % (uint32_t)cam.width), ly = (int)(id / (uint32_t)cam.width);
            r = camera_ray(cam, x, tile_global_row(tile, ly), rng);
            depth = 0, first_counted = false;
            trav_begin(T, r.org, ray_dir(r), stack);
            if constexpr (kSkip) origin_skip_none(stack);
            live = true, waiting = false;
        }
        if (!(REQ ? drained : exhausted)) {
            const unsigned long long idle_m = __ballot(!live && !waiting);
            const uint32_t cnt = (uint32_t)__popcll(idle_m);
            if (cnt >= refill.threshold()) {
                if (chunk_pos == chunk_end) {
                    if (!exhausted) {
                        uint32_t w = SLICED ? SliceCursor::claim_width(cnt, n) : !REQ && n_samples > 1u ? cnt : chunk_slots;
                        if (tail_guided) {
                            const uint32_t left = n > seen ? n - seen : 0u;
                            const uint32_t share = (uint32_t)(((unsigned long long)left * inv_waves) >> 16);
                            const uint32_t least = cnt > 16u ? cnt : 16u;
                            if (share < w) w = share > least ? share : least;
                        }
                        uint32_t base = 0;
                        if (lane == 0) base = atomicAdd(cursor, w);
                        base = (uint32_t)__builtin_amdgcn_readfirstlane((int)base) + n_waves * first_slots;
                        seen = base + w;
                        if (base >= n_total) {
                            exhausted = true;
                        } else {
                            chunk_pos = base;
                            chunk_end = base + w < n_total ? base + w : n_total;
                        }
                    }
                    if (REQ && exhausted) {
                        const uint32_t w = cnt > kRqClaim ? cnt : kRqClaim;
                        uint32_t h = 0;
                        if (lane == 0) h = atomicAdd(fq.ctl + 32, w);
                        h = (uint32_t)__builtin_amdgcn_readfirstlane((int)h);
                        if (h >= total_entries) {
                            drained = true;
                        } else {
                            chunk_pos = h;
                            chunk_end = h + w < total_entries ? h + w : total_entries;
                            chunk_dq = true;
                        }
                    }
                }
                if (chunk_pos != chunk_end) {
                    const uint32_t avail = chunk_end - chunk_pos;
                    const uint32_t take = cnt < avail ? cnt : avail;
                    const uint32_t rank = lane_rank(idle_m);
                    uint32_t first_here = 0, first_next = 0;
                    if (SLICED) {
                        slice_j = SliceCursor::advance(slice_j, n_slices, chunk_pos, n);
                        if (slice_j) first_here = frame_slice_bound(slices, slice_j - 1u);
                        first_next = frame_slice_bound(slices, slice_j);
                    }
                    if (!live && !waiting && rank < take) {
                        if (REQ && chunk_dq) {
                            id = chunk_pos + rank;
                            waiting = true;
                        } else {
                            uint32_t slot = chunk_pos + rank, first = 0;
                            if (SLICED) {
                                const SliceSlot m = SliceCursor::map(slot, slice_j, n, first_here, first_next);
                                slot = m.slot, first = m.first;
                            }
                            if (SLICED && slot >= n) {
                                slot_lost = 1u;
                            } else {
                                id = queue_load(qin, slot, r);
                                if (SLICED && first != 0u) {
                                    depth = kPend;
                                    samples_left = n_samples - first, first_counted = false;
                                    live = true;
                                } else if (!(holes && id == kNoRay)) {
                                    rng = rng_buf[id];
                                    depth = first_depth;
                                    samples_left = n_samples, first_counted = !holes;
                                    if (SLICED && CARRY) {
                                        const float4 a = accum[id];
                                        *sum_r = a.x, *sum_g = a.y, *sum_b = a.z;
                                    } else if (SLICED) {
                                        *sum_r = 0.0f, *sum_g = 0.0f, *sum_b = 0.0f;
                                    }
                                    if (!REQ && n_samples > 1u && xg_packed) {
                                        const uint32_t w = (uint32_t)camp->width;
                                        *xg_word() = (id % w) | ((uint32_t)tile_global_row(tile, (int)(id / w)) << 16);
                                    }
                                    trav_begin(T, r.org, ray_dir(r), stack);
                                    if constexpr (kSkip) origin_skip_none(stack);
                                    live = true;
                                }
                            }
                        }
                    }
                    chunk_pos += take;
                }
            }
        }
        const unsigned long long wait_m = REQ ? __ballot(waiting) : 0ull;
        if (REQ && waiting) {
            const unsigned long long e64 = rq_load64(fq.entries + id);
            samples_left = (uint32_t)e64, rng = (uint32_t)(e64 >> 32);
        }
        const uint32_t n_live = (uint32_t)__popcll(__ballot(live));
        if (n_live == 0) {
            if (!REQ) {
                if (exhausted) break;
                continue;
            }
            if (staged) flush();
            if (wait_m != 0ull) {
                if (++idle_polls > kRqIdleCap) {
                    if (lane == 0) __hip_atomic_store(fq.error, 1u, __ATOMIC_RELAXED, __HIP_MEMORY_SCOPE_AGENT);
                    break;
                }
                __builtin_amdgcn_s_sleep(8);
                continue;
            }
            if (drained) break;
            continue;
        }
        idle_polls = 0;
        const TravSigns sg = trav_signs(T);
        const lmask live_m = lanes(live);
        const uint32_t n_rays = SLICED ? count(live_m & lanes(depth < kPend)) : n_live;
        const uint32_t shade_at = n_rays * kMegaShadePct + (n_live - n_rays) * 100u;
        for (;;) {
            const lmask done = trav_done(T);
            if (count(done & live_m) * 100u >= shade_at) break;
            if (STATS) ws.live_lane_steps += n_live * kFinishUnroll;
            refill.stepped();
            (void)trav_step_wave<STATS, true, kSkip>(S, T, stack, top, sg, trav_classes(T, done), &ws);
#pragma unroll
            for (int k = 1; k < kFinishUnroll; ++k) (void)trav_step_wave<STATS, true, kSkip>(S, T, stack, top, sg, &ws);
        }
        if (STATS) ws.shade_rounds++, ws.shade_lanes += (uint32_t)__popcll(__ballot(live && T.cur == kTravDone));
        __builtin_amdgcn_s_setprio(0);
        bool requeue = false, slot_finished = false, hand_on = false;
        {
            const unsigned long long traced = __ballot(live && T.cur == kTravDone && !(SLICED && depth >= kPend));
            wave_rays += (unsigned long long)__popcll(__ballot(live && T.cur == kTravDone && !(first_counted && depth == first_depth) && !(SLICED && depth >= kPend)));
            if (SLICED && traced == 0ull && __ballot(live && depth < kPend) == 0ull && slice_wait_count(slice_looks_word(sum_r, (lds_f32_t*)sum_lds), slices) && lane == 0 && fq.error)
                __hip_atomic_store(fq.error, 4u, __ATOMIC_RELAXED, __HIP_MEMORY_SCOPE_AGENT);
        }
        if (SLICED && live && T.cur == kTravDone && depth >= kPend) {
            const SliceNow sn = frame_slices(slices);
            const auto rsrc = state_rsrc(sn);
            const uint32_t at = id * 32u, tag = sn.head.z + (n_samples - samples_left);
            const u32x4 w0 = __builtin_amdgcn_raw_buffer_load_b128(rsrc, (int)at, 0, 16 );
            const u32x4 w1 = __builtin_amdgcn_raw_buffer_load_b128(rsrc, (int)(at + 16u), 0, 16 );
            if ((w0.y == tag && w0.w == tag && w1.y == tag && w1.w == tag) || slice_wait_over(slice_looks_word(sum_r, (lds_f32_t*)sum_lds), slices)) {
                *sum_r = __uint_as_float(w0.x), *sum_g = __uint_as_float(w0.z), *sum_b = __uint_as_float(w1.x);
                rng = w1.z;
                const CameraDev cam = *camp;
                int x, gy;
                if (xg_packed) {
                    const uint32_t xg = *xg_word();
                    x = (int)(xg & 0xFFFFu), gy = (int)(xg >> 16);
                } else {
                    x = (int)(id % (uint32_t)cam.width), gy = tile_global_row(tile, (int)(id / (uint32_t)cam.width));
                }
                r = camera_ray(cam, x, gy, rng);
                depth = 0;
                trav_begin(T, r.org, ray_dir(r), stack);
                if constexpr (kSkip) origin_skip_none(stack);
            }
        } else if (live && T.cur == kTravDone) {
            f3 res;
            const bool done = shade_bounce<true>(S, rng, r, T.best, res, &T, &tab);
            depth++;
            bool ends = done;
            bool bounced = !done;
            if (SLICED && done) {
                *sum_r = *sum_r + clamp01(res.x), *sum_g = *sum_g + clamp01(res.y), *sum_b = *sum_b + clamp01(res.z);
            } else if (done) {
                float4 acc;
                if (REQ) {
                    const u32x4 a = __builtin_amdgcn_raw_buffer_load_b128(accum_rsrc, (int)(id * 16u), 0, 16 );
                    acc = make_float4(__uint_as_float(a.x), __uint_as_float(a.y), __uint_as_float(a.z), __uint_as_float(a.w));
                } else {
                    acc = accum[id];
                }
                acc.x = acc.x + clamp01(res.x), acc.y = acc.y + clamp01(res.y), acc.z = acc.z + clamp01(res.z);
                if (REQ) {
                    u32x4 a;
                    a.x = __float_as_uint(acc.x), a.y = __float_as_uint(acc.y), a.z = __float_as_uint(acc.z), a.w = __float_as_uint(acc.w);
                    __builtin_amdgcn_raw_buffer_store_b128(a, accum_rsrc, (int)(id * 16u), 0, 16 );
                } else {
                    accum[id] = acc;
                }
            } else if (depth == max_depth) {
                ends = true;
            } else if (rr_start && depth >= rr_start) {
                ends = !roulette(rng, r);
            }
            bool handed = false;
            if (SLICED && ends && samples_left > 1u) {
                const SliceNow sn = frame_slices(slices);
                const unsigned long long cuts = ((unsigned long long)sn.cuts.y << 32) | sn.cuts.x;
                const uint32_t sh = sn.head.w, s_next = n_samples - (samples_left - 1u);
                handed = (s_next & ((1u << sh) - 1u)) == 0u && ((cuts >> (s_next >> sh)) & 1ull) != 0ull;
                if (handed) {
                    const auto rsrc = state_rsrc(sn);
                    const uint32_t at = id * 32u, tag = sn.head.z + s_next;
                    u32x4 w0, w1;
                    w0.x = __float_as_uint(*sum_r), w0.y = tag, w0.z = __float_as_uint(*sum_g), w0.w = tag;
                    w1.x = __float_as_uint(*sum_b), w1.y = tag, w1.z = rng, w1.w = tag;
                    __builtin_amdgcn_raw_buffer_store_b128(w0, rsrc, (int)at, 0, 16 );
                    __builtin_amdgcn_raw_buffer_store_b128(w1, rsrc, (int)(at + 16u), 0, 16 );
                }
            }
            if (!REQ && ends && !handed && --samples_left) {
                const CameraDev cam = *camp;
                int x, gy;
                if (xg_packed) {
                    const uint32_t xg = *xg_word();
                    x = (int)(xg & 0xFFFFu), gy = (int)(xg >> 16);
                } else {
                    x = (int)(id % (uint32_t)cam.width), gy = tile_global_row(tile, (int)(id / (uint32_t)cam.width));
                }
                r = camera_ray(cam, x, gy, rng);
                depth = 0, first_counted = false;
                ends = false, bounced = false;
            }
            if (ends && !handed && cost_out) cost_out[id] = (uint8_t)(depth < 255u ? depth : 255u);
            if (SLICED && ends && !handed) accum[id] = make_float4(*sum_r, *sum_g, *sum_b, 0.0f);
            if (ends) {
                live = false, slot_finished = true;
                if (REQ) requeue = samples_left > 1u;
                if (!requeue && !handed) rng_buf[id] = rng;
            } else if (LIMIT && depth - first_depth >= bounce_limit) {
                hand_on = true, live = false, slot_finished = true;
            } else {
                const uint32_t from = bounced ? T.best.tri : kNoTri;
                trav_begin(T, r.org, ray_dir(r), stack);
                if constexpr (kSkip) origin_skip(S, from, T, stack);
            }
        }
        if (LIMIT) {
            const unsigned long long hm = __ballot(hand_on);
            if (hm != 0ull) {
                const uint32_t n_req = (uint32_t)__popcll(hm);
                uint32_t b0 = 0, c0 = 0, b1 = 0;
                if (lane == 0) {
                    for (;;) {
                        const unsigned long long old = atomicAdd(&out_word, (unsigned long long)n_req);
                        const uint32_t used = (uint32_t)old, base = (uint32_t)(old >> 32);
                        if (used + n_req <= kOutBlock) {
                            b0 = base + used, c0 = n_req;
                            break;
                        }
                        if (used <= kOutBlock) {
                            b0 = base + used, c0 = kOutBlock - used;
                            b1 = atomicAdd(count_out, kOutBlock);
                            __hip_atomic_store(&out_word, ((unsigned long long)b1 << 32) | (unsigned long long)(n_req - c0), __ATOMIC_RELAXED, __HIP_MEMORY_SCOPE_WORKGROUP);
                            break;
                        }
                        uint32_t polls = 0;
                        while ((uint32_t)__hip_atomic_load(&out_word, __ATOMIC_RELAXED, __HIP_MEMORY_SCOPE_WORKGROUP) > kOutBlock && ++polls < kRqIdleCap)
                            __builtin_amdgcn_s_sleep(1);
                        if (polls >= kRqIdleCap) {
                            if (fq.error) __hip_atomic_store(fq.error, 3u, __ATOMIC_RELAXED, __HIP_MEMORY_SCOPE_AGENT);
                            b0 = 0, c0 = n_req;
                            break;
                        }
                    }
                }
                b0 = (uint32_t)__builtin_amdgcn_readfirstlane((int)b0), c0 = (uint32_t)__builtin_amdgcn_readfirstlane((int)c0);
                b1 = (uint32_t)__builtin_amdgcn_readfirstlane((int)b1);
                const uint32_t rank = lane_rank(hm);
                if (hand_on) {
                    queue_store(qout, rank < c0 ? b0 + rank : b1 + (rank - c0), id, r);
                    rng_buf[id] = rng;
                }
            }
        }
        refill.round(slot_finished);
        if (REQ) {
            const unsigned long long rq_m = __ballot(requeue);
            const uint32_t n_rq = (uint32_t)__popcll(rq_m);
            if (n_rq) {
                const uint32_t rank = lane_rank(rq_m);
                if (requeue) stage[staged + rank] = (unsigned long long)(id | ((samples_left - 2u) << 24)) | ((unsigned long long)rng << 32);
                staged += n_rq;
            }
            stale = staged ? stale + 1u : 0u;
            if (staged >= kRqFlush || (staged && (wait_m != 0ull || stale >= 4u))) flush(), stale = 0;
        }
        __builtin_amdgcn_s_setprio(2);
    }
    if (SLICED && lane == 0 && slot_lost && fq.error) __hip_atomic_store(fq.error, 5u, __ATOMIC_RELAXED, __HIP_MEMORY_SCOPE_AGENT);
    if (lane == 0 && wave_rays) atomicAdd(extra_rays, wave_rays);
    if (STATS && lane == 0) wave_stats_flush(ws, stats_out);
    leave();
}

template <bool CARRY = false>
__global__ void __launch_bounds__(256) k_wf_resolve(uint32_t n_local, uint32_t spp, uint32_t width, uint32_t strip_rows,
                                                     uint32_t n_lanes, uint32_t lane_index, const float4* __restrict__ accum,
                                                     float* __restrict__ out_f32, uint8_t* __restrict__ out_u8,
                                                     const uint32_t* __restrict__ rng, u32x4* __restrict__ carry) {
    const uint32_t i = blockIdx.x * 256u + threadIdx.x;
    if (i >= n_local) return;
    const float4 a = accum[i];
    const uint32_t x = i % width, row = stream_lane_row(i / width, strip_rows, n_lanes, lane_index);
    const size_t o = (size_t)row * width + x;
    pixel_end(&a.x, &a.y, &a.z, (float)spp, o, out_f32, out_u8);
    if (CARRY) carry[o] = carry_word(a.x, a.y, a.z, rng[i]);
}


__global__ void __launch_bounds__(256) k_blocks_begin(const uint32_t* __restrict__ list, uint32_t n_blocks, uint32_t blocks_x, uint32_t width,
                                                       uint32_t local_rows, uint32_t samples, const u32x4* __restrict__ carry, u32x4* __restrict__ snap,
                                                       uint32_t* __restrict__ count, uint32_t* __restrict__ snap_count) {
    const uint32_t i = blockIdx.x * 4u + (threadIdx.x >> 6), w = threadIdx.x & 63u;
    if (i >= n_blocks) return;
    const uint32_t b = list ? list[i] : i;
    const uint32_t x = (b % blocks_x) * 8u + (w & 7u), ly = (b / blocks_x) * 8u + (w >> 3);
    if (x < width && ly < local_rows) snap[(size_t)ly * width + x] = carry[(size_t)ly * width + x];
    if (w == 0) {
        const uint32_t c = count[b];
        snap_count[b] = c;
        count[b] = c + samples;
    }
}

__global__ void __launch_bounds__(256) k_blocks_resolve(uint32_t n_local, uint32_t width, uint32_t blocks_x, const u32x4* __restrict__ carry,
                                                         const uint32_t* __restrict__ count, float* __restrict__ out_f32, uint8_t* __restrict__ out_u8) {
    const uint32_t i = blockIdx.x * 256u + threadIdx.x;
    if (i >= n_local) return;
    const uint32_t x = i % width, ly = i / width;
    const u32x4 a = carry[i];
    const float sr = __uint_as_float(a.x), sg = __uint_as_float(a.y), sb = __uint_as_float(a.z);
    pixel_end(&sr, &sg, &sb, (float)count[(ly >> 3) * blocks_x + (x >> 3)], i, out_f32, out_u8);
}

__global__ void __launch_bounds__(256) k_wf_generate_blocks(const CameraDev* __restrict__ camp, TileDev tile, const uint32_t* __restrict__ list,
                                                             uint32_t n_blocks, uint32_t tile_rows, uint32_t strip_rows, uint32_t n_lanes,
                                                             uint32_t lane_index, uint32_t* __restrict__ rng, QueueDev q,
                                                             uint32_t* __restrict__ count_out) {
    const uint32_t i = blockIdx.x * 256u + threadIdx.x;
    const CameraDev cam = *camp;
    const uint32_t width = (uint32_t)cam.width, blocks_x = (width + 7u) >> 3;
    bool take = false;
    uint32_t id = 0;
    if (i < n_blocks * 64u) {
        const uint32_t b = list[i >> 6], w = i & 63u;
        const uint32_t x = (b % blocks_x) * 8u + (w & 7u), row = (b / blocks_x) * 8u + (w >> 3);
        const uint32_t strip = row / strip_rows;
        if (x < width && row < tile_rows && strip % n_lanes == lane_index) {
            id = ((strip / n_lanes) * strip_rows + row % strip_rows) * width + x;
            take = true;
        }
    }
    const unsigned long long m = __ballot(take);
    if (m == 0ull) return;
    uint32_t base = 0;
    if ((threadIdx.x & 63u) == 0u) base = atomicAdd(count_out, (uint32_t)__popcll(m));
    base = (uint32_t)__builtin_amdgcn_readfirstlane((int)base);
    if (!take) return;
    const uint32_t rank = lane_rank(m);
    const int x = (int)(id % width), gy = tile_global_row(tile, (int)(id / width));
    uint32_t st = rng[id];
    const RayState r = gy < cam.height ? camera_ray(cam, x, gy, st) : RayState{};
    rng[id] = st;
    queue_store(q, base + rank, id, r);
}

__global__ void __launch_bounds__(256) k_wf_resolve_blocks(uint32_t n_local, uint32_t width, uint32_t strip_rows, uint32_t n_lanes, uint32_t lane_index,
                                                            const uint32_t* __restrict__ count, const float4* __restrict__ accum,
                                                            float* __restrict__ out_f32, uint8_t* __restrict__ out_u8,
                                                            const uint32_t* __restrict__ rng, u32x4* __restrict__ carry) {
    const uint32_t i = blockIdx.x * 256u + threadIdx.x;
    if (i >= n_local) return;
    const float4 a = accum[i];
    const uint32_t x = i % width, row = stream_lane_row(i / width, strip_rows, n_lanes, lane_index);
    const size_t o = (size_t)row * width + x;
    pixel_end(&a.x, &a.y, &a.z, (float)count[(row >> 3) * ((width + 7u) >> 3) + (x >> 3)], o, out_f32, out_u8);
    carry[o] = carry_word(a.x, a.y, a.z, rng[i]);
}

constexpr float kAdaptEps = 1e-4f;
__global__ void __launch_bounds__(256) k_adapt_errors(uint32_t n_blocks, uint32_t blocks_x, uint32_t width, uint32_t local_rows,
                                                       const u32x4* __restrict__ carry, const u32x4* __restrict__ snap,
                                                       const uint32_t* __restrict__ count, const uint32_t* __restrict__ snap_count, float threshold,
                                                       uint32_t min_samples, float* __restrict__ err, uint32_t* __restrict__ active) {
    const uint32_t b = blockIdx.x * 4u + (threadIdx.x >> 6), w = threadIdx.x & 63u;
    if (b >= n_blocks) return;
    const uint32_t n = count[b], n0 = snap_count[b];
    const uint32_t x = (b % blocks_x) * 8u + (w & 7u), ly = (b / blocks_x) * 8u + (w >> 3);
    const bool in = x < width && ly < local_rows;
    float e = 0.0f;
    if (in && n0 != 0u) {
        const size_t o = (size_t)ly * width + x;
        const u32x4 c = carry[o], a = snap[o];
        const float fn = (float)n, fa = (float)n0;
        const float ir = __uint_as_float(c.x) / fn, ig = __uint_as_float(c.y) / fn, ib = __uint_as_float(c.z) / fn;
        const float ar = __uint_as_float(a.x) / fa, ag = __uint_as_float(a.y) / fa, ab = __uint_as_float(a.z) / fa;
        e = (__builtin_fabsf(ir - ar) + __builtin_fabsf(ig - ag) + __builtin_fabsf(ib - ab)) / __builtin_sqrtf(kAdaptEps + ir + ig + ib);
    }
#pragma unroll
    for (int off = 32; off > 0; off >>= 1) e += __shfl_xor(e, off, 64);
    const uint32_t n_in = (uint32_t)__popcll(__ballot(in));
    if (w == 0) {
        const float eb = n0 != 0u ? e / (float)n_in : __builtin_inff();
        err[b] = eb;
        active[b] = n0 == 0u || n < min_samples || eb >= threshold ? 1u : 0u;
    }
}

__global__ void __launch_bounds__(1024) k_adapt_compact(uint32_t n_blocks, const uint32_t* __restrict__ active, uint32_t* __restrict__ out) {
    __shared__ uint32_t wave_n[16];
    const uint32_t lane = threadIdx.x & 63u, wv = threadIdx.x >> 6;
    uint32_t base = 0;
    for (uint32_t c = 0; c < n_blocks; c += 1024u) {
        const uint32_t i = c + threadIdx.x;
        const bool f = i < n_blocks && active[i] != 0u;
        const unsigned long long m = __ballot(f);
        if (lane == 0) wave_n[wv] = (uint32_t)__popcll(m);
        __syncthreads();
        uint32_t before = 0, total = 0;
        for (uint32_t k = 0; k < 16u; ++k) {
            const uint32_t v = wave_n[k];
            before += k < wv ? v : 0u;
            total += v;
        }
        const uint32_t rank = lane_rank(m);
        if (f) out[1u + base + before + rank] = i;
        base += total;
        __syncthreads();
    }
    if (threadIdx.x == 0) out[0] = base;
}

}
```

sycl-ray-tracer_amd/csrc/rt_scene_image.h:

```cpp
#pragma once
#include <algorithm>
#include <cmath>
#include <cstring>
#include <vector>

#include "scene_build.h"

namespace rt {

constexpr size_t kMaxDeviceNodes = 0x7FFFFFFF / sizeof(BvhNode);
inline std::vector<BvhNode> device_nodes(const std::vector<BvhNode>& host) {
    std::vector<BvhNode> dn(host);
    for (BvhNode& n : dn)
        for (int k = 0; k < 4; ++k) n.child[k] = (int32_t)device_child_word(n.child[k]);
    return dn;
}
inline void host_nodes(std::vector<BvhNode>& nodes) {
    for (BvhNode& n : nodes)
        for (int k = 0; k < 4; ++k) n.child[k] = host_child_word((uint32_t)n.child[k]);
}

constexpr size_t kTriTailBytes = 48;
static_assert(kTriBytes + kTriTailBytes >= 80 && kTriBytes <= sizeof(TriRec), "a last leaf of one record is read as five 16-byte loads too");
inline size_t packed_tri_bytes(size_t n_records) { return n_records * kTriBytes + kTriTailBytes; }
inline std::vector<uint8_t> pack_tris(const std::vector<TriRec>& tris) {
    std::vector<uint8_t> packed(packed_tri_bytes(tris.size()), 0);
    for (size_t r = 0; r < tris.size(); ++r) std::memcpy(packed.data() + r * kTriBytes, &tris[r], kTriBytes);
    return packed;
}
inline void unpack_tris(const std::vector<uint8_t>& packed, std::vector<TriRec>& tris) {
    for (size_t r = 0; r < tris.size(); ++r) std::memcpy(&tris[r], packed.data() + r * kTriBytes, kTriBytes);
}

inline void scene_scalars(const HostScene& hs, SceneDev& dev) {
    dev.n_nodes = (uint32_t)hs.nodes.size();
    dev.n_tris = (uint32_t)(hs.wverts.size() / 9);
    std::memcpy(dev.sky, hs.sky, 12);
    dev.packed_mat = hs.packed_mat ? 1u : 0u;
    const bool stage = hs.packed_mat && hs.n_layers <= 65536u;
    dev.lds_nm = stage ? (uint32_t)std::min<size_t>(hs.inst.size(), kLdsNm) : 0u;
    dev.lds_mats = stage ? (uint32_t)std::min<size_t>(hs.mats.size(), kLdsMats) : 0u;
    for (int a = 0; a < 3; ++a) {
        const float ext = hs.bounds_hi[a] - hs.bounds_lo[a];
        dev.cell_lo[a] = hs.bounds_lo[a];
        dev.cell_scale[a] = ext > 0.0f && std::isfinite(ext) ? 4.0f / ext : 0.0f;
    }
}

}
```

sycl-ray-tracer_amd/csrc/rt_types.h:

```cpp
#pragma once
#include <cstddef>
#include <cstdint>

namespace rt {

#ifdef __HIPCC__
#define RT_HD __host__ __device__ inline
#else
#define RT_HD inline
#endif
struct alignas(64) BvhNode {
    float origin[3];
    float scale_x;
    uint32_t q[6];
    float scale_y, scale_z;
    int32_t child[4];
    RT_HD float scale(int a) const { const float s = a == 0 ? scale_x : (a == 1 ? scale_y : scale_z); return s < 0.0f ? -s : s; }
    RT_HD void set_scale(int a, float s) { (a == 0 ? scale_x : (a == 1 ? scale_y : scale_z)) = s; }
};
static_assert(sizeof(BvhNode) == 64, "BvhNode must be 64 bytes");
constexpr int32_t kChildEmpty = (int32_t)0x80000000;
struct Box3 {
    float lo[3], hi[3];
};

RT_HD void clear_planes(BvhNode& n) {
    n.scale_x = n.scale_y = n.scale_z = 1.0f;
    n.origin[0] = n.origin[1] = n.origin[2] = 0.0f;
    for (int i = 0; i < 6; ++i) n.q[i] = (i & 1) ? 0u : 0xFFFFFFFFu;
}
RT_HD BvhNode empty_node() {
    BvhNode n;
    clear_planes(n);
    for (int k = 0; k < 4; ++k) n.child[k] = kChildEmpty;
    return n;
}
struct LeafRange {
    uint32_t first, count;
};
RT_HD LeafRange leaf_range(int32_t child) {
    const uint32_t code = (uint32_t)~child;
    return {code >> 2, (code & 3u) + 1u};
}
RT_HD int32_t leaf_child(uint32_t first, uint32_t count) { return ~(int32_t)((first << 2) | (count - 1)); }
RT_HD float child_plane(const BvhNode& n, int k, int a, int side) { return n.origin[a] + (float)((n.q[2 * a + side] >> (8 * k)) & 0xffu) * n.scale(a); }
RT_HD Box3 child_box(const BvhNode& n, int k) {
    Box3 b;
    for (int a = 0; a < 3; ++a) b.lo[a] = child_plane(n, k, a, 0), b.hi[a] = child_plane(n, k, a, 1);
    return b;
}

RT_HD uint32_t device_child_word(int32_t child) { return child >= 0 ? (uint32_t)child * 64u : (uint32_t)child; }
RT_HD int32_t host_child_word(uint32_t word) { return (int32_t)word >= 0 ? (int32_t)(word / 64u) : (int32_t)word; }
constexpr int kMaxLeafTris = 2;
constexpr int kTopNodes = 341;
constexpr int kStackSize = 64;
constexpr uint32_t kNoTri = 0xFFFFFFFFu;
constexpr float kTNear = 0.0001f;

struct ContractRange {
    float lo[3], hi[3];
    float limit;
    uint32_t finite_only;
};
RT_HD float contract_max(float a, float b) { return a < b ? b : a; }
RT_HD bool in_contract_range(const ContractRange& r, float ox, float oy, float oz) {
    if (r.finite_only) return __builtin_isfinite(ox) && __builtin_isfinite(oy) && __builtin_isfinite(oz);
    const float o[3] = {ox, oy, oz};
    for (int a = 0; a < 3; ++a) {
        const float outside = contract_max(contract_max(r.lo[a] - o[a], o[a] - r.hi[a]), 0.0f);
        if (!(outside <= r.limit)) return false;
    }
    return true;
}

struct alignas(16) TriRec {
    float v0[3];
    float e1[3];
    float e2[3];
    uint32_t global_index;
    uint32_t pad[2];
};
static_assert(sizeof(TriRec) == 48, "TriRec must be 48 bytes");
constexpr uint32_t kTriBytes = 40;
RT_HD const float* packed_tri(const uint8_t* tris, size_t r) { return reinterpret_cast<const float*>(tris + r * kTriBytes); }
RT_HD float* packed_tri(uint8_t* tris, size_t r) { return reinterpret_cast<float*>(tris + r * kTriBytes); }
RT_HD uint32_t packed_global_index(const uint8_t* tris, size_t r) { return reinterpret_cast<const uint32_t*>(tris + r * kTriBytes)[9]; }

constexpr uint32_t kPackedInstBits = 20, kPackedInstMask = (1u << kPackedInstBits) - 1u;
struct alignas(64) ShadeRec {
    float n0[3], n1[3], n2[3];
    float uv0[2], uv1[2], uv2[2];
    uint32_t instance;
};
static_assert(sizeof(ShadeRec) == 64, "ShadeRec must be 64 bytes");

constexpr uint32_t kLdsNm = 8, kLdsMats = 24;
struct alignas(16) InstRec {
    float normal_mat[9];
    uint32_t material;
    uint32_t pad[2];
};
static_assert(sizeof(InstRec) == 48, "InstRec must be 48 bytes");

struct alignas(16) MatRec {
    uint32_t type;
    uint32_t tex_kind;
    float color[3];
    uint32_t tex_layer;
    float emissive[3];
    float roughness;
    float ior;
    uint32_t pad;
};
static_assert(sizeof(MatRec) == 48, "MatRec must be 48 bytes");

constexpr uint32_t kSkipNone = 1u;
constexpr float kSkipDist = 40400.0f;
constexpr float kSkipTilt = 1.0f / 256.0f;
struct alignas(16) SkipRec {
    uint32_t ref;
    float n[3];
    float p[3];
    uint32_t a;
};
static_assert(sizeof(SkipRec) == 32, "SkipRec must be 32 bytes");
RT_HD float skip_half(uint32_t bits16) {
    const uint16_t b = (uint16_t)bits16;
    _Float16 h;
    __builtin_memcpy(&h, &b, 2);
    return (float)h;
}
RT_HD uint32_t origin_skip_word(const SkipRec& e, const float o[3], const float d[3]) {
    const float wx = o[0] - e.p[0], wy = o[1] - e.p[1], wz = o[2] - e.p[2];
    const float s = __builtin_fmaf(e.n[2], wz, __builtin_fmaf(e.n[1], wy, e.n[0] * wx));
    const float nd = __builtin_fabsf(__builtin_fmaf(e.n[2], d[2], __builtin_fmaf(e.n[1], d[1], e.n[0] * d[0])));
    const float l = (__builtin_fabsf(wx) + __builtin_fabsf(wy)) + __builtin_fabsf(wz);
    const float ld = (__builtin_fabsf(d[0]) + __builtin_fabsf(d[1])) + __builtin_fabsf(d[2]);
    const float thr = __builtin_fmaf(skip_half(e.a >> 16), l, __builtin_fmaf(kSkipDist, __builtin_fabsf(s), skip_half(e.a & 0xffffu)));
    return (nd > thr && nd > kSkipTilt * ld) ? e.ref : kSkipNone;
}

struct SceneDev {
    const BvhNode* nodes;
    const uint8_t* tris;
    const ShadeRec* shade;
    const InstRec* inst;
    const MatRec* mats;
    const uint8_t* tex;
    uint32_t n_nodes;
    uint32_t n_tris;
    float sky[3];
    float cell_lo[3], cell_scale[3];
    uint32_t packed_mat;
    uint32_t lds_nm, lds_mats;
    const SkipRec* skip;
};

struct CameraDev {
    float center[3], pixel00[3], du[3], dv[3];
    int32_t width, height;
};

struct TileDev {
    uint32_t rank, world, strip_rows;
    int32_t local_rows;
};

}
```

sycl-ray-tracer_amd/csrc/rt_update.hip:

```cpp
#include "rt_internal.h"
#include "rt_scene_image.h"
#include "scene_rules.h"

#include <algorithm>
#include <limits>

namespace rtlib {
namespace {

__host__ __device__ inline uint32_t order_key(float f) {
    uint32_t b;
    std::memcpy(&b, &f, 4);
    if (f == 0.0f) b = 0u;
    return (b & 0x80000000u) ? ~b : (b | 0x80000000u);
}
__device__ __forceinline__ unsigned long long min_key(float f, uint32_t v) {
    return ((unsigned long long)order_key(f) << 32) | (unsigned long long)((v << 1) | (__float_as_uint(f) >> 31));
}
__device__ __forceinline__ unsigned long long max_key(float f, uint32_t v) {
    return ((unsigned long long)order_key(f) << 32) | (unsigned long long)(((~v & 0x3FFFFFFFu) << 1) | (__float_as_uint(f) >> 31));
}
inline float key_value(unsigned long long key) {
    const uint32_t k = (uint32_t)(key >> 32);
    uint32_t b = (k & 0x80000000u) ? (k & 0x7FFFFFFFu) : ~k;
    if (b == 0u && (key & 1ull)) b = 0x80000000u;
    float f;
    std::memcpy(&f, &b, 4);
    return f;
}

constexpr uint32_t kRedWords = 8;

template <bool WRITE = true>
__global__ void __launch_bounds__(256) k_upd_transform(uint32_t n_tris, const float* __restrict__ pos, const uint32_t* __restrict__ idx,
                                                        const uint32_t* __restrict__ tri_inst, const float* __restrict__ xf,
                                                        float* __restrict__ wv, unsigned long long* __restrict__ red) {
    const uint32_t t = blockIdx.x * 256u + threadIdx.x;
    unsigned long long kmin[3] = {~0ull, ~0ull, ~0ull}, kmax[3] = {0ull, 0ull, 0ull};
    uint32_t bad = 0;
    if (t < n_tris) {
        const float* m = xf + 16 * (size_t)tri_inst[t];
        for (int k = 0; k < 3; ++k) {
            const uint32_t vi = idx[3 * (size_t)t + k];
            const float x = pos[3 * (size_t)vi], y = pos[3 * (size_t)vi + 1], z = pos[3 * (size_t)vi + 2];
            for (int a = 0; a < 3; ++a) {
                const float p = world_coord(m, a, x, y, z);
                if (WRITE) wv[9 * (size_t)t + 3 * k + a] = p;
                bad |= isfinite(p) ? 0u : 1u;
                const uint32_t v = 3u * t + (uint32_t)k;
                kmin[a] = min(kmin[a], min_key(p, v));
                kmax[a] = max(kmax[a], max_key(p, v));
            }
        }
    }
    for (int off = 32; off > 0; off >>= 1) {
        for (int a = 0; a < 3; ++a) {
            kmin[a] = min(kmin[a], (unsigned long long)__shfl_xor(kmin[a], off));
            kmax[a] = max(kmax[a], (unsigned long long)__shfl_xor(kmax[a], off));
        }
        bad |= (uint32_t)__shfl_xor((int)bad, off);
    }
    __shared__ unsigned long long s_key[4][6];
    __shared__ uint32_t s_bad[4];
    const uint32_t lane = threadIdx.x & 63u, wave = threadIdx.x >> 6;
    if (lane == 0) {
        for (int a = 0; a < 3; ++a) s_key[wave][a] = kmin[a], s_key[wave][3 + a] = kmax[a];
        s_bad[wave] = bad;
    }
    __syncthreads();
    if (threadIdx.x == 0) {
        for (int w = 1; w < 4; ++w) {
            for (int a = 0; a < 3; ++a) kmin[a] = min(kmin[a], s_key[w][a]), kmax[a] = max(kmax[a], s_key[w][3 + a]);
            bad |= s_bad[w];
        }
        for (int a = 0; a < 3; ++a) atomicMin(&red[a], kmin[a]), atomicMax(&red[3 + a], kmax[a]);
        if (bad) atomicOr(&red[6], 1ull);
    }
}

__global__ void __launch_bounds__(256) k_upd_records(uint32_t n_recs, uint8_t* __restrict__ tris, const float* __restrict__ wv) {
    const uint32_t r = blockIdx.x * 256u + threadIdx.x;
    if (r >= n_recs) return;
    const uint32_t g = packed_global_index(tris, r);
    if (g == kNoTri) return;
    float* rec = packed_tri(tris, r);
    tri_record(wv + 9 * (size_t)g, rec, rec + 3, rec + 6);
}

__global__ void __launch_bounds__(128) k_upd_refit(uint32_t n, const uint32_t* __restrict__ level, BvhNode* __restrict__ nodes,
                                                    const uint8_t* __restrict__ tris, const float* __restrict__ wv, Box3* __restrict__ box,
                                                    float pad, unsigned long long* __restrict__ failed) {
    const uint32_t i = blockIdx.x * 128u + threadIdx.x;
    if (i >= n) return;
    const uint32_t ni = level[i];
    const BvhNode nd = nodes[ni];
    BvhNode q;
    const RefitResult res = refit_node(
        nd, [=](int32_t child) { return box[host_child_word((uint32_t)child)]; },
        [=](uint32_t r) { return wv + 9 * (size_t)packed_global_index(tris, r); }, pad, box[ni], q);
    if (res == kRefitEmpty) return;
    if (res == kRefitRefused) atomicOr(failed, 1ull);
    nodes[ni] = q;
}

__global__ void __launch_bounds__(256) k_upd_words(uint32_t n_tris, const uint32_t* __restrict__ tri_inst, const uint32_t* __restrict__ islot,
                                                    ShadeRec* __restrict__ shade) {
    const uint32_t t = blockIdx.x * 256u + threadIdx.x;
    if (t >= n_tris) return;
    const uint32_t w = islot[tri_inst[t]];
    if (shade[t].instance != w) shade[t].instance = w;
}

__global__ void __launch_bounds__(256) k_upd_normals(uint32_t n_tris, const uint32_t* __restrict__ idx, const float* __restrict__ nrm,
                                                      ShadeRec* __restrict__ shade) {
    const uint32_t t = blockIdx.x * 256u + threadIdx.x;
    if (t >= n_tris) return;
    shade_normals(shade[t], idx + 3 * (size_t)t, nrm);
}

std::vector<float> transforms_of(const rt_instance* inst, size_t n) {
    std::vector<float> xf(16 * n);
    for (size_t i = 0; i < n; ++i) std::memcpy(&xf[16 * i], inst[i].transform, 64);
    return xf;
}

void commit_update(rt_scene* s, const std::vector<rt_instance>& inst, const std::vector<uint32_t>& slot, const rt_update_stats& done, rt_update_stats* stats) {
    s->upd->inst_slot = slot, s->upd->instances = inst, s->upd->host_stale = s->device >= 0;
    if (stats) *stats = done;
}

int update_host(rt_scene* s, const std::vector<rt_instance>& inst, const rt_scene_update_desc* u, rt_update_stats* stats) {
    SceneUpdate& up = *s->upd;
    HostScene& hs = s->hs;
    const uint32_t T = (uint32_t)up.tri_instance.size();
    const bool new_pos = u->n_vertices && u->positions, new_nrm = u->n_vertices && u->normals;
    std::vector<float> wv;
    world_vertices(T, up.indices.data(), up.tri_instance.data(), inst.data(), new_pos ? u->positions : up.positions.data(), wv);
    float lo[3] = {0, 0, 0}, hi[3] = {0, 0, 0}, pad = hs.pad;
    std::string err;
    if (T && !world_bounds(wv, lo, hi, pad, err)) return fail(RT_ERR_INVALID, err);
    HostScene next = hs;
    if (T) {
        next.wverts.swap(wv);
        std::memcpy(next.bounds_lo, lo, 12), std::memcpy(next.bounds_hi, hi, 12);
        next.pad = pad;
        std::vector<float> box;
        if (!refit_host(next, up.level_nodes, box, err)) return fail(RT_ERR_INVALID, err);
    }
    std::vector<uint32_t> slot;
    shading_rows(inst.data(), (uint32_t)inst.size(), up.inst_use, hs.packed_mat, next.inst, slot);
    for (uint32_t t = 0; t < T; ++t) {
        const uint32_t i = up.tri_instance[t];
        next.shade[t].instance = shading_word(hs.packed_mat, slot[i], inst[i].material, i);
        if (new_nrm) shade_normals(next.shade[t], &up.indices[3 * (size_t)t], u->normals);
    }
    hs = std::move(next);
    if (new_pos) up.positions.assign(u->positions, u->positions + 3 * (size_t)up.n_vertices);
    if (new_nrm) up.normals.assign(u->normals, u->normals + 3 * (size_t)up.n_vertices);
    commit_update(s, inst, slot, rt_update_stats{0.0, 0u, T ? (uint32_t)up.level_nodes.size() : 0u}, stats);
    return RT_OK;
}

template <bool WRITE>
void launch_transform(const SceneUpdate& up, uint32_t T, const float* pos, const float* xf) {
    hipLaunchKernelGGL(k_upd_transform<WRITE>, dim3((T + 255u) / 256u), dim3(256), 0, up.stream, T, pos, (const uint32_t*)up.d_idx.get(),
                       (const uint32_t*)up.d_tri_inst.get(), xf, up.d_wv.get(), up.d_red.get());
}

int update_device(rt_scene* s, const std::vector<rt_instance>& inst, const rt_scene_update_desc* u, rt_update_stats* stats) {
    SceneUpdate& up = *s->upd;
    HostScene& hs = s->hs;
    HIPCHK(hipSetDevice(s->device));
    const uint32_t T = (uint32_t)(hs.wverts.size() / 9), I = (uint32_t)inst.size();
    const uint32_t n_recs = s->dev.n_tris ? (uint32_t)hs.tris.size() : 0u;
    const uint32_t g256 = (T + 255u) / 256u;
    hipStream_t st = up.stream;
    unsigned long long* h_red = up.h_red.get();
    rt_update_stats done{};
    HIPCHK(hipEventRecord(up.ev0, st));
    const bool new_xf = u->n_instances != 0, new_pos = u->n_vertices && u->positions, new_nrm = u->n_vertices && u->normals;
    const std::vector<float> xf = new_xf ? transforms_of(inst.data(), I) : std::vector<float>();
    if (new_xf) HIPCHK(hipMemcpyAsync(up.d_xf_stage.get(), xf.data(), xf.size() * 4, hipMemcpyHostToDevice, st));
    if (new_pos) HIPCHK(hipMemcpyAsync(up.d_pos_stage.get(), u->positions, 12 * (size_t)up.n_vertices, hipMemcpyHostToDevice, st));
    const float* xf_new = new_xf ? up.d_xf_stage.get() : up.d_xf.get();
    const float* pos_new = new_pos ? up.d_pos_stage.get() : up.d_pos.get();
    float lo[3] = {0, 0, 0}, hi[3] = {0, 0, 0}, pad = hs.pad;
    if (T) {
        for (int a = 0; a < 3; ++a) h_red[a] = ~0ull, h_red[3 + a] = 0ull;
        h_red[6] = h_red[7] = 0ull;
        HIPCHK(hipMemcpyAsync(up.d_red.get(), h_red, kRedWords * 8, hipMemcpyHostToDevice, st));
        if (up.keep_previous) launch_transform<false>(up, T, pos_new, xf_new);
        else launch_transform<true>(up, T, pos_new, xf_new);
        ++done.launches;
        HIPCHK(hipGetLastError());
        HIPCHK(hipMemcpyAsync(h_red, up.d_red.get(), kRedWords * 8, hipMemcpyDeviceToHost, st));
        HIPCHK(hipStreamSynchronize(st));
        for (int a = 0; a < 3; ++a) lo[a] = key_value(h_red[a]), hi[a] = key_value(h_red[3 + a]);
        std::string err;
        const bool ok = h_red[6] == 0 ? scene_padding(lo, hi, pad, err) : (err = "non-finite world-space vertex", false);
        if (!ok && up.keep_previous) return fail(RT_ERR_INVALID, err);
        if (!ok) {
            launch_transform<true>(up, T, up.d_pos.get(), up.d_xf.get());
            HIPCHK(hipGetLastError());
            HIPCHK(hipStreamSynchronize(st));
            return fail(RT_ERR_INVALID, err);
        }
        if (up.keep_previous) {
            std::swap(up.d_wv, up.d_wv_prev);
            launch_transform<true>(up, T, pos_new, xf_new);
            ++done.launches;
            HIPCHK(hipGetLastError());
        }
    }
    if (new_xf) std::swap(up.d_xf, up.d_xf_stage);
    if (new_pos) std::swap(up.d_pos, up.d_pos_stage);
    if (T) {
        hipLaunchKernelGGL(k_upd_records, dim3((n_recs + 255u) / 256u), dim3(256), 0, st, n_recs, s->d_tris.get(), (const float*)up.d_wv.get());
        ++done.launches;
        h_red[7] = 0ull;
        HIPCHK(hipMemcpyAsync(up.d_red.get() + 7, h_red + 7, 8, hipMemcpyHostToDevice, st));
        for (size_t h = 0; h + 1 < up.level_start.size(); ++h) {
            const uint32_t n = up.level_start[h + 1] - up.level_start[h];
            if (!n) continue;
            hipLaunchKernelGGL(k_upd_refit, dim3((n + 127u) / 128u), dim3(128), 0, st, n, (const uint32_t*)(up.d_levels.get() + up.level_start[h]),
                               s->d_nodes.get(), (const uint8_t*)s->d_tris.get(), (const float*)up.d_wv.get(), (Box3*)up.d_box.get(), pad, up.d_red.get() + 7);
            ++done.launches;
            done.refit_nodes += n;
        }
        HIPCHK(hipGetLastError());
    }
    std::vector<InstRec> rows;
    std::vector<uint32_t> slot, words;
    shading_rows(inst.data(), I, up.inst_use, hs.packed_mat, rows, slot);
    const bool moved = slot != up.inst_slot;
    if (new_xf) {
        if (rows.size() > scene_inst_capacity(s)) return fail(RT_ERR_INVALID, "internal: instance table capacity exceeded");
        HIPCHK(hipMemcpyAsync(s->d_inst.get(), rows.data(), rows.size() * sizeof(InstRec), hipMemcpyHostToDevice, st));
    }
    if (moved && T) {
        words.resize(I);
        for (uint32_t i = 0; i < I; ++i) words[i] = shading_word(hs.packed_mat, slot[i], inst[i].material, i);
        HIPCHK(hipMemcpyAsync(up.d_islot.get(), words.data(), (size_t)I * 4, hipMemcpyHostToDevice, st));
        hipLaunchKernelGGL(k_upd_words, dim3(g256), dim3(256), 0, st, T, (const uint32_t*)up.d_tri_inst.get(), (const uint32_t*)up.d_islot.get(), s->d_shade.get());
        ++done.launches;
    }
    if (new_nrm && T) {
        HIPCHK(hipMemcpyAsync(up.d_pos_stage.get(), u->normals, 12 * (size_t)up.n_vertices, hipMemcpyHostToDevice, st));
        hipLaunchKernelGGL(k_upd_normals, dim3(g256), dim3(256), 0, st, T, (const uint32_t*)up.d_idx.get(), (const float*)up.d_pos_stage.get(), s->d_shade.get());
        ++done.launches;
    }
    HIPCHK(hipGetLastError());
    HIPCHK(hipEventRecord(up.ev1, st));
    HIPCHK(hipStreamSynchronize(st));
    if (T) HIPCHK(hipMemcpy(h_red + 7, up.d_red.get() + 7, 8, hipMemcpyDeviceToHost));
    float ms = 0.0f;
    HIPCHK(hipEventElapsedTime(&ms, up.ev0, up.ev1));
    done.device_ms = (double)ms;
    commit_update(s, inst, slot, done, stats);
    if (T && h_red[7]) {
        ++s->generation;
        return fail(RT_ERR_INVALID, "internal: a refit node's child boxes could not be quantised");
    }
    hs.inst = rows;
    if (T) std::memcpy(hs.bounds_lo, lo, 12), std::memcpy(hs.bounds_hi, hi, 12), hs.pad = pad;
    scene_scalars(hs, s->dev);
    return RT_OK;
}

}

uint32_t scene_inst_capacity(const rt_scene* s) {
    return (uint32_t)std::max<size_t>(std::max<size_t>(s->hs.inst.size(), s->upd ? s->upd->instances.size() : 0), 1);
}

int init_scene_update(rt_scene* s, const rt_scene_desc* d, bool keep_previous) {
    s->upd.reset(new SceneUpdate());
    SceneUpdate& u = *s->upd;
    u.keep_previous = keep_previous;
    const uint32_t T = d->n_triangles, I = d->n_instances, V = d->n_vertices;
    u.n_vertices = V;
    u.instances.assign(d->instances, d->instances + I);
    u.inst_use.assign(I, 0);
    for (uint32_t t = 0; t < T; ++t) u.inst_use[d->tri_instance[t]]++;
    {
        std::vector<InstRec> rows;
        shading_rows(d->instances, I, u.inst_use, s->hs.packed_mat, rows, u.inst_slot);
    }
    node_levels(s->hs.nodes, u.level_nodes, u.level_start);
    if (s->device < 0) {
        if (T) {
            u.positions.assign(d->positions, d->positions + 3 * (size_t)V);
            u.normals.assign(d->normals, d->normals + 3 * (size_t)V);
        }
        u.indices.assign(d->indices, d->indices + 3 * (size_t)T);
        u.tri_instance.assign(d->tri_instance, d->tri_instance + T);
        return RT_OK;
    }
    HIPCHK(hipSetDevice(s->device));
    SceneAlloc& al = s->alloc;
    uint64_t& b = s->device_bytes;
    const size_t n_nodes = s->hs.nodes.size();
    const float* wv = T ? s->hs.wverts.data() : nullptr;
    const std::vector<float> xf = transforms_of(d->instances, I);
    int rc = u.d_pos.upload(al, T ? d->positions : nullptr, 3 * (size_t)V, b);
    if (!rc) rc = u.d_pos_stage.upload(al, nullptr, 3 * (size_t)V, b);
    if (!rc) rc = u.d_idx.upload(al, d->indices, 3 * (size_t)T, b);
    if (!rc) rc = u.d_tri_inst.upload(al, d->tri_instance, T, b);
    if (!rc) rc = u.d_xf.upload(al, xf, b);
    if (!rc) rc = u.d_xf_stage.upload(al, nullptr, xf.size(), b);
    if (!rc) rc = u.d_islot.upload(al, nullptr, I, b);
    if (!rc) rc = u.d_wv.upload(al, wv, 9 * (size_t)T, b);
    if (!rc && keep_previous && T) rc = u.d_wv_prev.upload(al, wv, 9 * (size_t)T, b);
    if (!rc) rc = u.d_box.upload(al, nullptr, 6 * n_nodes, b);
    if (!rc) rc = u.d_levels.upload(al, u.level_nodes, b);
    if (!rc) rc = u.d_red.upload(al, nullptr, kRedWords, b);
    if (rc) return rc;
    HIPCHK(al.pinned((void**)&u.h_red.p, kRedWords * 8));
    HIPCHK(hipStreamCreateWithFlags(&u.stream, hipStreamNonBlocking));
    HIPCHK(hipEventCreate(&u.ev0));
    HIPCHK(hipEventCreate(&u.ev1));
    HIPCHK(hipMemset(u.d_box.get(), 0, 24 * std::max<size_t>(n_nodes, 1)));
    return RT_OK;
}

int sync_host_copy(const rt_scene* cs) {
    rt_scene* s = const_cast<rt_scene*>(cs);
    if (!s->upd || !s->upd->host_stale) return RT_OK;
    return no_throw([&]() -> int {
        SceneUpdate& up = *s->upd;
        HostScene& hs = s->hs;
        HIPCHK(hipSetDevice(s->device));
        std::vector<BvhNode> nodes(hs.nodes.size());
        std::vector<uint8_t> packed(packed_tri_bytes(hs.tris.size()));
        std::vector<float> wv(hs.wverts.size()), box(6 * hs.nodes.size());
        std::vector<ShadeRec> shade(hs.shade.size());
        HIPCHK(hipMemcpy(nodes.data(), s->d_nodes.get(), nodes.size() * sizeof(BvhNode), hipMemcpyDeviceToHost));
        HIPCHK(hipMemcpy(packed.data(), s->d_tris.get(), packed.size(), hipMemcpyDeviceToHost));
        if (!wv.empty()) HIPCHK(hipMemcpy(wv.data(), up.d_wv.get(), wv.size() * 4, hipMemcpyDeviceToHost));
        HIPCHK(hipMemcpy(box.data(), up.d_box.get(), box.size() * 4, hipMemcpyDeviceToHost));
        if (!shade.empty()) HIPCHK(hipMemcpy(shade.data(), s->d_shade.get(), shade.size() * sizeof(ShadeRec), hipMemcpyDeviceToHost));
        host_nodes(nodes);
        unpack_tris(packed, hs.tris);
        hs.nodes.swap(nodes);
        hs.wverts.swap(wv);
        hs.shade.swap(shade);
        record_boxes(hs);
        if (!hs.wverts.empty()) hs.sah_cost = refit_sah_cost(hs, box);
        up.host_stale = false;
        return (int)RT_OK;
    });
}

}

extern "C" int rt_scene_update(rt_scene* s, const rt_scene_update_desc* u, rt_update_stats* stats) {
    if (!s || !u) return fail(RT_ERR_INVALID, "null argument");
    if (!s->upd) return fail(RT_ERR_INVALID, "the scene was not created updatable (rt_scene_create_ex with RT_SCENE_UPDATABLE)");
    if (s->frames_pending) return fail(RT_ERR_INVALID, "a renderer of the scene has a frame in flight (rt_render_frame_end first)");
    const SceneUpdate& up = *s->upd;
    if (u->n_instances && u->n_instances != up.instances.size()) return fail(RT_ERR_INVALID, "n_instances must be 0 or the scene's");
    if (u->n_instances && !u->instances) return fail(RT_ERR_INVALID, "null instance array");
    if (u->n_vertices && u->n_vertices != up.n_vertices) return fail(RT_ERR_INVALID, "n_vertices must be 0 or the scene's");
    if (u->n_vertices && !u->positions && !u->normals) return fail(RT_ERR_INVALID, "n_vertices given with neither positions nor normals");
    for (uint32_t i = 0; i < u->n_instances; ++i)
        if (u->instances[i].material != up.instances[i].material) return fail(RT_ERR_INVALID, "an update cannot change an instance's material");
    if (!s->readers.empty()) {
        HIPCHK(hipSetDevice(s->device));
        for (const auto& se : s->readers) HIPCHK(hipEventSynchronize(se.second));
    }
    return no_throw([&]() -> int {
        std::vector<rt_instance> inst = up.instances;
        for (uint32_t i = 0; i < u->n_instances; ++i) inst[i] = u->instances[i];
        rt_update_stats local{};
        const int rc = s->device < 0 ? update_host(s, inst, u, &local) : update_device(s, inst, u, &local);
        if (rc != RT_OK) return rc;
        ++s->generation;
        if (stats) *stats = local;
        return (int)RT_OK;
    });
}
```

Before: 10720.

## Scale ray parameter by a power of two to fold slab clamp into FMA

Rays in the main kernels now have their inverse direction and hit distance scaled by a scene-dependent power of two (2^-near_k, chosen from the scene bounds). Every in-scene distance then falls below 1, so the z-slab entry term in the box test can use a single `v_fma_f32 ... clamp` in place of an FMA followed by a max with zero. Triangle hit t is scaled the same way so it compares against box distances, and shading unscales t before moving the ray origin. The exponent reaches the device through the TopTree limit field and a scalar OR trick. This adds complexity and precision/edge-case risk, for example for rays starting outside the bounds or very large distances. The unused n_tris field is replaced by near_k.

```diff
diff --git a/sycl-ray-tracer_amd/csrc/rt_bounce.h b/sycl-ray-tracer_amd/csrc/rt_bounce.h
--- a/sycl-ray-tracer_amd/csrc/rt_bounce.h
+++ b/sycl-ray-tracer_amd/csrc/rt_bounce.h
@@ -5,14 +5,14 @@
 
 RT_DEV f3 ray_dir(const RayState& r) { return mk3(h2f(r.dir[0]), h2f(r.dir[1]), h2f(r.dir[2])); }
 
-template <bool FROM_TRAV = false, class Sink = NoSink>
+template <bool FROM_TRAV = false, bool SCALED = false, class Sink = NoSink>
 RT_DEV bool shade_bounce(const SceneDev& S, uint32_t& rng, RayState& r, const Hit& h, f3& result, const Trav* T = nullptr, const ShadeTables* tab = nullptr,
-                         long long* ck = nullptr, const Sink& sink = Sink{}) {
+                         long long* ck = nullptr, const Sink& sink = Sink{}, int32_t lim = 0) {
     f3 org = FROM_TRAV ? T->o : r.org;
     f3 dir = FROM_TRAV ? T->d : ray_dir(r);
     f3 att = mk3(h2f(r.att[0]), h2f(r.att[1]), h2f(r.att[2]));
     f3 rad = mk3(h2f(r.rad[0]), h2f(r.rad[1]), h2f(r.rad[2]));
-    const bool done = FROM_TRAV ? shade_hit<true>(S, *tab, rng, h, org, dir, att, rad, result, ck, sink) : shade_hit<false>(S, ShadeTables{}, rng, h, org, dir, att, rad, result, nullptr, sink);
+    const bool done = FROM_TRAV ? shade_hit<true, Sink, SCALED>(S, *tab, rng, h, org, dir, att, rad, result, ck, sink, lim) : shade_hit<false>(S, ShadeTables{}, rng, h, org, dir, att, rad, result, nullptr, sink);
     r.org = org;
     r.dir[0] = f2h(dir.x), r.dir[1] = f2h(dir.y), r.dir[2] = f2h(dir.z);
     r.att[0] = f2h(att.x), r.att[1] = f2h(att.y), r.att[2] = f2h(att.z);
diff --git a/sycl-ray-tracer_amd/csrc/rt_device.h b/sycl-ray-tracer_amd/csrc/rt_device.h
--- a/sycl-ray-tracer_amd/csrc/rt_device.h
+++ b/sycl-ray-tracer_amd/csrc/rt_device.h
@@ -120,7 +120,15 @@
 RT_DEV f3 cross3f(f3 a, f3 b) {
     return mk3(__builtin_fmaf(a.y, b.z, -(a.z * b.y)), __builtin_fmaf(a.z, b.x, -(a.x * b.z)), __builtin_fmaf(a.x, b.y, -(a.y * b.x)));
 }
-RT_DEV void tri_test_regs(float4 a, float4 b, float2 c, f3 o, f3 d, Hit& best) {
+RT_DEV int32_t near_exp(int32_t lim) {
+    int32_t e;
+    asm volatile("s_or_b32 %0, %1, -64" : "=s"(e) : "s"(lim) : "scc");
+    return e;
+}
+RT_DEV float near_scale(int32_t lim) { return __uint_as_float((uint32_t)(127 + near_exp(lim)) << 23); }
+RT_DEV float near_unscale(int32_t lim) { return __uint_as_float((uint32_t)(127 - near_exp(lim)) << 23); }
+template <bool SCALED = false>
+RT_DEV void tri_test_regs(float4 a, float4 b, float2 c, f3 o, f3 d, Hit& best, int32_t lim = 0) {
     const f3 v0 = mk3(a.x, a.y, a.z), e1 = mk3(a.w, b.x, b.y), e2 = mk3(b.z, b.w, c.x);
     const uint32_t gidx = __float_as_uint(c.y);
     const f3 p = cross3f(d, e2);
@@ -133,8 +141,9 @@
     const float un = un0 * sgn, vn = vn0 * sgn;
     if (!(un >= 0.0f && vn >= 0.0f && un + vn <= __builtin_fabsf(det))) return;
     const float inv = rcp_rn(det);
-    const float t = dot3f(e2, q) * inv;
-    if (!(t > kTNear)) return;
+    const float t1 = dot3f(e2, q) * inv;
+    if (!(t1 > kTNear)) return;
+    const float t = SCALED ? t1 * near_scale(lim) : t1;
     if (t < best.t || (t == best.t && gidx < best.tri)) {
         best.t = t;
         best.u = un0 * inv;
@@ -173,7 +182,8 @@
 
 struct TravStack;
 RT_DEV uint32_t stack_base(const TravStack& st);
-RT_DEV void trav_begin(Trav& T, f3 o, f3 d, const TravStack& st) {
+template <bool SCALED = false>
+RT_DEV void trav_begin(Trav& T, f3 o, f3 d, const TravStack& st, int32_t lim = 0) {
     T.o = o, T.d = d;
     T.best.t = __builtin_huge_valf();
     T.best.u = T.best.v = 0.0f;
@@ -183,6 +193,10 @@
     const float dy = __builtin_fabsf(d.y) < kTiny ? __builtin_copysignf(kTiny, d.y) : d.y;
     const float dz = __builtin_fabsf(d.z) < kTiny ? __builtin_copysignf(kTiny, d.z) : d.z;
     T.ix = __builtin_amdgcn_rcpf(dx), T.iy = __builtin_amdgcn_rcpf(dy), T.iz = __builtin_amdgcn_rcpf(dz);
+    if (SCALED) {
+        const float t_s = near_scale(lim);
+        T.ix *= t_s, T.iy *= t_s, T.iz *= t_s;
+    }
     T.ox = -o.x * T.ix, T.oy = -o.y * T.iy, T.oz = -o.z * T.iz;
     T.cur = 0;
     T.sp = stack_base(st);
@@ -224,6 +238,7 @@
     lds_u32x4* w2;
     lds_u32x4* ch;
     int32_t count;
+    int32_t lim;
 };
 RT_DEV void top_tree_fill(const SceneDev& S, u32x4* w0, u32x4* w1, u32x4* w2, u32x4* ch, int32_t count) {
     for (int32_t i = (int32_t)threadIdx.x; i < count; i += (int32_t)blockDim.x) {
@@ -265,15 +280,20 @@
     uint32_t inner_steps = 0, inner_lanes = 0, leaf_steps = 0, leaf_lanes = 0;
     uint32_t shade_rounds = 0, shade_lanes = 0, live_lane_steps = 0, top_lanes = 0;
 };
+RT_DEV float fma_clamp01(float a, float b, float c) {
+    float d;
+    asm("v_fma_f32 %0, %1, %2, %3 clamp" : "=v"(d) : "v"(a), "v"(b), "v"(c));
+    return d;
+}
 RT_DEV TravSigns trav_signs(const Trav& T) { return TravSigns{lanes(T.ix < 0.0f), lanes(T.iy < 0.0f), lanes(T.iz < 0.0f)}; }
-template <bool SKIP = false, bool MISS_KEYS = false>
+template <bool SKIP = false, bool MISS_KEYS = false, bool NEAR = false>
 RT_DEV void trav_inner(const SceneDev& S, Trav& T, const TravStack& stack, const TopTree& top, const TravSigns& sg) {
     const float inf = __builtin_huge_valf();
     uint32_t skip = kSkipNone;
     if (SKIP) skip = (uint32_t)*lds_at(skip_word_addr(stack));
     float k0, k1, k2, k3;
     u32x4 w0, w1, w2, chw;
-    if (T.cur < top.count * 64) {
+    if (T.cur < (NEAR ? top.lim : top.count * 64)) {
         const uint32_t o = (uint32_t)T.cur >> 2;
         w0 = *(lds_u32x4*)(size_t)((uint32_t)(size_t)top.w0 + o), w1 = *(lds_u32x4*)(size_t)((uint32_t)(size_t)top.w1 + o);
         w2 = *(lds_u32x4*)(size_t)((uint32_t)(size_t)top.w2 + o), chw = *(lds_u32x4*)(size_t)((uint32_t)(size_t)top.ch + o);
@@ -300,8 +320,9 @@
     lmask h0 = 0ull, h1 = 0ull, h2 = 0ull, h3 = 0ull;
 #define RT_CHILD(K, H, CVT, CW)                                                                           \
     {                                                                                                    \
-        const float tn = __builtin_fmaxf(__builtin_fmaxf(__builtin_fmaf(CVT(qnx), ax, bx), __builtin_fmaf(CVT(qny), ay, by)), \
-                                         __builtin_fmaxf(__builtin_fmaf(CVT(qnz), az, bz), 0.0f));       \
+        const float tn = NEAR ? __builtin_fmaxf(__builtin_fmaxf(__builtin_fmaf(CVT(qnx), ax, bx), __builtin_fmaf(CVT(qny), ay, by)), fma_clamp01(CVT(qnz), az, bz)) \
+                              : __builtin_fmaxf(__builtin_fmaxf(__builtin_fmaf(CVT(qnx), ax, bx), __builtin_fmaf(CVT(qny), ay, by)), \
+                                                __builtin_fmaxf(__builtin_fmaf(CVT(qnz), az, bz), 0.0f)); \
          \
          \
          \
@@ -381,8 +402,8 @@
     }
 }
 
-template <bool BATCH>
-RT_DEV void trav_leaf(const SceneDev& S, Trav& T, const TravStack& stack) {
+template <bool BATCH, bool SCALED = false>
+RT_DEV void trav_leaf(const SceneDev& S, Trav& T, const TravStack& stack, int32_t lim = 0) {
     const uint32_t code = (uint32_t)~T.cur;
     const uint32_t first = code >> 2, rem = code & 3u;
     if (BATCH) {
@@ -390,9 +411,9 @@
         const uint8_t* p4 = S.tris + (size_t)first * kTriBytes;
         const float4 l0 = tri_ld4(p4), l1 = tri_ld4(p4 + 16), l2 = tri_ld4(p4 + 32), l3 = tri_ld4(p4 + 48), l4 = tri_ld4(p4 + 64);
         const bool two = rem != 0u;
-        tri_test_regs(l0, l1, make_float2(l2.x, l2.y), T.o, T.d, T.best);
+        tri_test_regs<SCALED>(l0, l1, make_float2(l2.x, l2.y), T.o, T.d, T.best, lim);
         if (__ballot(two) != 0ull) {
-            if (two) tri_test_regs(make_float4(l2.z, l2.w, l3.x, l3.y), make_float4(l3.z, l3.w, l4.x, l4.y), make_float2(l4.z, l4.w), T.o, T.d, T.best);
+            if (two) tri_test_regs<SCALED>(make_float4(l2.z, l2.w, l3.x, l3.y), make_float4(l3.z, l3.w, l4.x, l4.y), make_float2(l4.z, l4.w), T.o, T.d, T.best, lim);
         }
         if (lanes(!stack_shallow(stack, T, 0u)) == 0ull) trav_pop_lds(T, stack);
         else trav_pop(T, stack);
@@ -412,21 +433,21 @@
     const lmask inner = lanes(T.cur >= 0);
     return TravClasses{inner, lanes(true) & ~(inner | done)};
 }
-template <bool STATS = false, bool LEAF_BATCH = false, bool SKIP = false, bool MISS_KEYS = false>
+template <bool STATS = false, bool LEAF_BATCH = false, bool SKIP = false, bool MISS_KEYS = false, bool NEAR = false>
 RT_DEV uint32_t trav_step_wave(const SceneDev& S, Trav& T, const TravStack& stack, const TopTree& top, const TravSigns& sg, const TravClasses& c, WaveStats* ws = nullptr) {
     const uint32_t ni = count(c.inner), nl = count(c.leaf);
     if (ni * kVoteInner >= nl * kVoteLeaf && !(LEAF_BATCH && nl >= 64u)) {
         if (STATS && ni) ws->inner_steps++, ws->inner_lanes += ni, ws->top_lanes += count(c.inner & lanes(T.cur < (SKIP ? top.count : kTopNodes) * 64));
-        if (in_mask(c.inner)) trav_inner<SKIP, MISS_KEYS>(S, T, stack, top, sg);
+        if (in_mask(c.inner)) trav_inner<SKIP, MISS_KEYS, NEAR>(S, T, stack, top, sg);
     } else {
         if (STATS) ws->leaf_steps++, ws->leaf_lanes += nl;
-        if (in_mask(c.leaf)) trav_leaf<LEAF_BATCH>(S, T, stack);
+        if (in_mask(c.leaf)) trav_leaf<LEAF_BATCH, NEAR>(S, T, stack, top.lim);
     }
     return ni + nl;
 }
-template <bool STATS = false, bool LEAF_BATCH = false, bool SKIP = false, bool MISS_KEYS = false>
+template <bool STATS = false, bool LEAF_BATCH = false, bool SKIP = false, bool MISS_KEYS = false, bool NEAR = false>
 RT_DEV uint32_t trav_step_wave(const SceneDev& S, Trav& T, const TravStack& stack, const TopTree& top, const TravSigns& sg, WaveStats* ws = nullptr) {
-    return trav_step_wave<STATS, LEAF_BATCH, SKIP, MISS_KEYS>(S, T, stack, top, sg, trav_classes(T), ws);
+    return trav_step_wave<STATS, LEAF_BATCH, SKIP, MISS_KEYS, NEAR>(S, T, stack, top, sg, trav_classes(T), ws);
 }
 
 RT_DEV Hit intersect(const SceneDev& S, f3 o, f3 d, const TravStack& stack, const TopTree& top) {
@@ -559,9 +580,9 @@
 struct NoSink {};
 template <class Sink> struct is_no_sink { static constexpr bool value = false; };
 template <> struct is_no_sink<NoSink> { static constexpr bool value = true; };
-template <bool USE_TAB = false, class Sink = NoSink>
+template <bool USE_TAB = false, class Sink = NoSink, bool SCALED = false>
 RT_DEV bool shade_hit(const SceneDev& S, const ShadeTables& tab, uint32_t& rng, const Hit& h, f3& org, f3& dir, f3& att, f3& rad, f3& result,
-                      long long* ck = nullptr, const Sink& sink = Sink{}) {
+                      long long* ck = nullptr, const Sink& sink = Sink{}, int32_t lim = 0) {
     if (h.tri == kNoTri) {
         if constexpr (is_no_sink<Sink>::value) result = att * (mk3(S.sky[0], S.sky[1], S.sky[2]) + rad);
         else sink(att * (mk3(S.sky[0], S.sky[1], S.sky[2]) + rad));
@@ -646,7 +667,8 @@
     const bool scattered = scatter<true>(S, mat, rng, d, normal, tu, tv, sdir, satt, texel);
     RT_STAMP_AFTER(ck, 4, satt.x);
     if (scattered) {
-        org = mk3(org.x + dir.x * h.t, org.y + dir.y * h.t, org.z + dir.z * h.t);
+        const float t = SCALED ? h.t * near_unscale(lim) : h.t;
+        org = mk3(org.x + dir.x * t, org.y + dir.y * t, org.z + dir.z * t);
         dir = sdir;
         att = att * satt;
         return false;
@@ -670,7 +692,7 @@
     const int32_t top_count = (int32_t)S.n_nodes < (NTOP) ? (int32_t)S.n_nodes : (NTOP);               \
     top_tree_fill(S, top_w0, top_w1, top_w2, top_ch, top_count);                                       \
     __syncthreads();                                                                                   \
-    const TopTree top{(lds_u32x4*)top_w0, (lds_u32x4*)top_w1, (lds_u32x4*)top_w2, (lds_u32x4*)top_ch, top_count}; \
+    const TopTree top{(lds_u32x4*)top_w0, (lds_u32x4*)top_w1, (lds_u32x4*)top_w2, (lds_u32x4*)top_ch, top_count, (EXTRA) ? top_count * 64 - (int32_t)S.near_k : 0}; \
     const TravStack stack{(uint32_t)(size_t)(lds_i32*)(lds_stack + threadIdx.x), spill, 4u * (BLOCK)}; \
     lds_stack[threadIdx.x] = kTravDone;
 
diff --git a/sycl-ray-tracer_amd/csrc/rt_kernels.h b/sycl-ray-tracer_amd/csrc/rt_kernels.h
--- a/sycl-ray-tracer_amd/csrc/rt_kernels.h
+++ b/sycl-ray-tracer_amd/csrc/rt_kernels.h
@@ -192,6 +192,7 @@
                                                     uint8_t* __restrict__ out_u8,
                                                     unsigned long long* __restrict__ ray_counter,
                                                     unsigned long long* __restrict__ stats_out, uint32_t n_slices) {
+    constexpr bool kNear = !((SLICED && CARRY == 1) || (!SLICED && CARRY == 2));
     WaveStats ws;
     long long t_begin = 0, t_mark = 0, t_trav = 0, t_shade = 0;
     long long ck[8] = {0, 0, 0, 0, 0, 0, 0, 0};
@@ -248,7 +249,7 @@
                     *color_r = 0.0f, *color_g = 0.0f, *color_b = 0.0f;
                     r = camera_ray(cam, x, gy, rng);
                 }
-                trav_begin(T, r.org, ray_dir(r), stack);
+                trav_begin<kNear>(T, r.org, ray_dir(r), stack, top.lim);
                 origin_skip_none(stack);
             } else {
                 depth = kPend;
@@ -309,9 +310,9 @@
             if (STATS >= 2) ws.live_lane_steps += n_live * (uint32_t)kMegaUnroll;
             if (STATS == 1) ws.inner_steps += (uint32_t)kMegaUnroll;
             refill.stepped();
-            (void)trav_step_wave<(STATS >= 2), true, true, true>(S, T, stack, top, sg, trav_classes(T, done), &ws);
+            (void)trav_step_wave<(STATS >= 2), true, true, true, kNear>(S, T, stack, top, sg, trav_classes(T, done), &ws);
 #pragma unroll
-            for (int k = 1; k < kMegaUnroll; ++k) (void)trav_step_wave<(STATS >= 2), true, true, true>(S, T, stack, top, sg, &ws);
+            for (int k = 1; k < kMegaUnroll; ++k) (void)trav_step_wave<(STATS >= 2), true, true, true, kNear>(S, T, stack, top, sg, &ws);
         }
         if (STATS) {
             ws.shade_rounds++;
@@ -348,9 +349,9 @@
                 const auto add = [color_r, color_g, color_b](const f3& c) { *color_r = *color_r + c.x, *color_g = *color_g + c.y, *color_b = *color_b + c.z; };
                 bool done;
                 if (SLICED) {
-                    done = shade_bounce<true>(S, rng, r, T.best, res, &T, &tab, STATS >= 2 ? ck : nullptr, add);
+                    done = shade_bounce<true, kNear>(S, rng, r, T.best, res, &T, &tab, STATS >= 2 ? ck : nullptr, add, top.lim);
                 } else {
-                    done = shade_bounce<true>(S, rng, r, T.best, res, &T, &tab, STATS >= 2 ? ck : nullptr);
+                    done = shade_bounce<true, kNear>(S, rng, r, T.best, res, &T, &tab, STATS >= 2 ? ck : nullptr, NoSink{}, top.lim);
                     if (done) add(res);
                 }
 #ifdef RT_TAIL_PRIO
@@ -402,7 +403,7 @@
             }
             if (live && depth < kPend) {
                 const uint32_t from = bounced ? T.best.tri : kNoTri;
-                trav_begin(T, r.org, ray_dir(r), stack);
+                trav_begin<kNear>(T, r.org, ray_dir(r), stack, top.lim);
                 origin_skip(S, from, T, stack);
             }
             RT_STAMP_AFTER((STATS >= 2 ? ck : nullptr), 5, T.ox);
@@ -733,6 +734,7 @@
     const uint32_t n_waves = gridDim.x * kWavesPerBlock;
     RT_SHADE_LDS
     constexpr bool kSkip = !LIMIT;
+    constexpr bool kNear = kSkip;
     RT_TRAVERSAL_LDS_SKIP(kMegaBlock, kSkip)
     __shared__ unsigned long long rq_stage_mem[REQ ? kWavesPerBlock * kRqStage : 1u];
     typedef __attribute__((address_space(3))) unsigned long long lds_u64_t;
@@ -822,7 +824,7 @@
             const int x = (int)(id % (uint32_t)cam.width), ly = (int)(id / (uint32_t)cam.width);
             r = camera_ray(cam, x, tile_global_row(tile, ly), rng);
             depth = 0, first_counted = false;
-            trav_begin(T, r.org, ray_dir(r), stack);
+            trav_begin<kNear>(T, r.org, ray_dir(r), stack, top.lim);
             if constexpr (kSkip) origin_skip_none(stack);
             live = true, waiting = false;
         }
@@ -906,7 +908,7 @@
                                         const uint32_t w = (uint32_t)camp->width;
                                         *xg_word() = (id % w) | ((uint32_t)tile_global_row(tile, (int)(id / w)) << 16);
                                     }
-                                    trav_begin(T, r.org, ray_dir(r), stack);
+                                    trav_begin<kNear>(T, r.org, ray_dir(r), stack, top.lim);
                                     if constexpr (kSkip) origin_skip_none(stack);
                                     live = true;
                                 }
@@ -950,9 +952,9 @@
             if (count(done & live_m) * 100u >= shade_at) break;
             if (STATS) ws.live_lane_steps += n_live * kFinishUnroll;
             refill.stepped();
-            (void)trav_step_wave<STATS, true, kSkip>(S, T, stack, top, sg, trav_classes(T, done), &ws);
+            (void)trav_step_wave<STATS, true, kSkip, false, kNear>(S, T, stack, top, sg, trav_classes(T, done), &ws);
 #pragma unroll
-            for (int k = 1; k < kFinishUnroll; ++k) (void)trav_step_wave<STATS, true, kSkip>(S, T, stack, top, sg, &ws);
+            for (int k = 1; k < kFinishUnroll; ++k) (void)trav_step_wave<STATS, true, kSkip, false, kNear>(S, T, stack, top, sg, &ws);
         }
         if (STATS) ws.shade_rounds++, ws.shade_lanes += (uint32_t)__popcll(__ballot(live && T.cur == kTravDone));
         __builtin_amdgcn_s_setprio(0);
@@ -982,12 +984,12 @@
                 }
                 r = camera_ray(cam, x, gy, rng);
                 depth = 0;
-                trav_begin(T, r.org, ray_dir(r), stack);
+                trav_begin<kNear>(T, r.org, ray_dir(r), stack, top.lim);
                 if constexpr (kSkip) origin_skip_none(stack);
             }
         } else if (live && T.cur == kTravDone) {
             f3 res;
-            const bool done = shade_bounce<true>(S, rng, r, T.best, res, &T, &tab);
+            const bool done = shade_bounce<true, kNear>(S, rng, r, T.best, res, &T, &tab, nullptr, NoSink{}, top.lim);
             depth++;
             bool ends = done;
             bool bounced = !done;
@@ -1053,7 +1055,7 @@
                 hand_on = true, live = false, slot_finished = true;
             } else {
                 const uint32_t from = bounced ? T.best.tri : kNoTri;
-                trav_begin(T, r.org, ray_dir(r), stack);
+                trav_begin<kNear>(T, r.org, ray_dir(r), stack, top.lim);
                 if constexpr (kSkip) origin_skip(S, from, T, stack);
             }
         }
diff --git a/sycl-ray-tracer_amd/csrc/rt_scene_image.h b/sycl-ray-tracer_amd/csrc/rt_scene_image.h
--- a/sycl-ray-tracer_amd/csrc/rt_scene_image.h
+++ b/sycl-ray-tracer_amd/csrc/rt_scene_image.h
@@ -34,7 +34,6 @@
 
 inline void scene_scalars(const HostScene& hs, SceneDev& dev) {
     dev.n_nodes = (uint32_t)hs.nodes.size();
-    dev.n_tris = (uint32_t)(hs.wverts.size() / 9);
     std::memcpy(dev.sky, hs.sky, 12);
     dev.packed_mat = hs.packed_mat ? 1u : 0u;
     const bool stage = hs.packed_mat && hs.n_layers <= 65536u;
@@ -45,6 +44,7 @@
         dev.cell_lo[a] = hs.bounds_lo[a];
         dev.cell_scale[a] = ext > 0.0f && std::isfinite(ext) ? 4.0f / ext : 0.0f;
     }
+    dev.near_k = near_clamp_exponent(hs.bounds_lo, hs.bounds_hi);
 }
 
 }
diff --git a/sycl-ray-tracer_amd/csrc/rt_types.h b/sycl-ray-tracer_amd/csrc/rt_types.h
--- a/sycl-ray-tracer_amd/csrc/rt_types.h
+++ b/sycl-ray-tracer_amd/csrc/rt_types.h
@@ -149,13 +149,22 @@
     const MatRec* mats;
     const uint8_t* tex;
     uint32_t n_nodes;
-    uint32_t n_tris;
+    uint32_t near_k;
     float sky[3];
     float cell_lo[3], cell_scale[3];
     uint32_t packed_mat;
     uint32_t lds_nm, lds_mats;
     const SkipRec* skip;
 };
+
+RT_HD uint32_t near_clamp_exponent(const float lo[3], const float hi[3]) {
+    float d = 0.0f;
+    for (int a = 0; a < 3; ++a) d += hi[a] > lo[a] ? hi[a] - lo[a] : 0.0f;
+    if (!(d > 0.0f)) return 1u;
+    uint32_t k = 1u;
+    while (k < 63u && !(d <= __builtin_ldexpf(1.0f, (int)k - 16))) ++k;
+    return k;
+}
 
 struct CameraDev {
     float center[3], pixel00[3], du[3], dv[3];
diff --git a/sycl-ray-tracer_amd/csrc/rt_update.hip b/sycl-ray-tracer_amd/csrc/rt_update.hip
--- a/sycl-ray-tracer_amd/csrc/rt_update.hip
+++ b/sycl-ray-tracer_amd/csrc/rt_update.hip
@@ -172,7 +172,7 @@
     HostScene& hs = s->hs;
     HIPCHK(hipSetDevice(s->device));
     const uint32_t T = (uint32_t)(hs.wverts.size() / 9), I = (uint32_t)inst.size();
-    const uint32_t n_recs = s->dev.n_tris ? (uint32_t)hs.tris.size() : 0u;
+    const uint32_t n_recs = T ? (uint32_t)hs.tris.size() : 0u;
     const uint32_t g256 = (T + 255u) / 256u;
     hipStream_t st = up.stream;
     unsigned long long* h_red = up.h_red.get();
```

Result: no change. 10820, median of 6 (+1.0%).
